# getanteon/alaz

Hardware: AMD Instinct MI355X
Metric: L7 edge-events/s ingested->scored service-map (higher is better)
Workload: dtype u64; 1 GPU; C3 device-resident replay: 10000 pods / 5000 services / 1000000 edges, 10000000 HTTP l7 events per window already in HBM, 2-layer SAGE + MLP score, partitioned K1 (variant 0, 8-byte records, 512 partitions); 2-batch HBM ring (value excludes PCIe: see end_to_end with --full); events_per_window=10000000, layers=2, windows_in_flight=1, parallelism=1 GPU

## Files before the change

alaz_amd/csrc/servicegraph.hip:

```cpp
#include <hip/hip_runtime.h>
#include <hip/hip_ext.h>

#include <algorithm>
#include <cmath>
#include <cstdio>
#include <cstring>
#include <chrono>
#include <condition_variable>
#include <thread>
#include <mutex>
#include <string>
#include <unordered_map>
#include <vector>

#include <dlfcn.h>

#include "join_host.hpp"
#include "sg_plan.hpp"
#include "sg_kernels.h"
#include "sg_sel.h"
#include "sg_trend.h"
#include "sg_node_trend.h"
#include "sg_rank.h"
#include "sg_incident.h"
// ... 160 lines not shown
    struct Impact { bool on = false; u32 max_hops = 0; sgplan::GroupImpactPlan plan; char* mem = nullptr; u32* pos = nullptr; u64* fresh = nullptr;
                    u64* next = nullptr; u64* ends = nullptr; u32* arrive = nullptr; u32* cnt = nullptr; u32* stage = nullptr; u32* stage_idx = nullptr;
                    std::vector<u64*> mask, rows, count; std::vector<u32*> hops; std::vector<char> valid; hipEvent_t ev = nullptr;
                    bool pending = false; } gimp;
    struct QuantSpace { bool on = false; char* mem = nullptr; u32* pos = nullptr; u32* tgt[2] = {nullptr, nullptr}; u64* part = nullptr;
                        unsigned char* stage = nullptr; u32* stage_idx = nullptr; std::vector<u64*> hist; std::vector<u32*> quant;
                        std::vector<char> valid; hipEvent_t ev = nullptr; bool pending = false; };
    struct Quantiles { sgplan::QuantPlan plan; u32 n_q = 0; u32 qm[SG_Q_MAX] = {}; QuantSpace sp[3]; } qnt;
    struct QuantTrend { u32 qi = 0; Baseline<sg_node_trend> nodes; Baseline<sg_edge_trend> groups; Baseline<sg_node_trend> workloads; } qtr;
    struct Traffic { double lat_floor = 0, err_floor = 0; Baseline<sg_edge_trend> edges; Baseline<sg_node_trend> nodes; Baseline<sg_edge_trend> groups;
                     Baseline<sg_node_trend> workloads; } trf;
};

namespace {

sg_engine::WinSlot& work(sg_engine* e) { return e->slots[e->cur]; }
int ran_slot(const sg_engine* e) { return e->last.slot >= 0 ? e->last.slot : e->cur; }
sg_engine::WinSlot& ran(sg_engine* e) { return e->slots[ran_slot(e)]; }

#define HIP_TRY(e, call)                                                                       \
    do {                                                                                       \
        hipError_t _r = (call);                                                                \
        if (_r != hipSuccess) {                                                                \
            (e)->err = std::string(#call) + ": " + hipGetErrorString(_r);                      \
            return _r == hipErrorOutOfMemory ? SG_ENOMEM : SG_ENODEV;                          \
        }                                                                                      \
    } while (0)

template <typename T>
int dev_alloc(sg_engine* e, T** p, size_t n, int fill = 0) {
    void* q = nullptr;
    size_t bytes = std::max<size_t>(n, 1) * sizeof(T);
    constexpr size_t kArenaMax = (size_t)32 << 20, kArenaChunk = (size_t)256 << 20, kArenaAlign = 4096;
    if (e->plan.arena_on && bytes < kArenaMax) {
        const size_t need = (bytes + kArenaAlign - 1) & ~(kArenaAlign - 1);
        if (need > e->arena_left) {
            void* c = nullptr;
            HIP_TRY(e, hipMalloc(&c, kArenaChunk));
            e->allocs.push_back(c);
            e->arena_base = static_cast<char*>(c); e->arena_left = kArenaChunk;
        }
        q = e->arena_base; e->arena_base += need; e->arena_left -= need;
    } else {
        HIP_TRY(e, hipMalloc(&q, bytes));
        e->allocs.push_back(q);
    }
    HIP_TRY(e, hipMemsetAsync(q, fill, bytes, e->slots[0].stream));
    *p = (T*)q;
    return SG_OK;
}

hipStream_t pick(sg_engine* e, void* s) { return s ? (hipStream_t)s : work(e).stream; }
hipStream_t pick_ran(sg_engine* e, void* s) { return s ? (hipStream_t)s : e->last.slot >= 0 ? e->last.stream : work(e).stream; }

hipEvent_t get_event(sg_engine* e) {
    if (!e->ev_pool.empty()) { hipEvent_t v = e->ev_pool.back(); e->ev_pool.pop_back(); return v; }
    hipEvent_t v; hipEventCreate(&v); return v;
}

struct Timed {
    sg_engine* e; hipStream_t s; TimingRec r; bool on;
    Timed(sg_engine* e_, hipStream_t s_, int kernel) : e(e_), s(s_), on(e_ && ((e_->timing >> kernel) & 1u)) {
        if (on) { r.kernel = kernel; r.a = get_event(e); r.b = get_event(e); hipEventRecord(r.a, s); }
    }
    ~Timed() { if (on) { hipEventRecord(r.b, s); e->trecs.push_back(r); } }
};

static_assert(sgplan::kK1bWarmU == K1B_WARM_U, "sg_plan.hpp's copy of pass B's warm U");
constexpr int k4_threads(int fi, bool proj, bool split) { return split ? (proj ? 512 : 256) : (fi == 32 ? 1024 : 512); }
template <class FnT, const auto& Keys> struct Family { typedef FnT Fn; static constexpr auto& keys = Keys; };
struct K1aWide : Family<K1aFn, sgplan::kK1aWideKeys> { template <size_t I> static Fn at() { constexpr auto k = keys[I]; return k1a_partition<(bool)k[0], (bool)k[1], (bool)k[2]>; } };
struct K1aTile : Family<K1aFn, sgplan::kK1aTileKeys> { template <size_t I> static Fn at() { constexpr auto k = keys[I]; return k1a_tile_partition<k[0], (bool)k[1], k[2]>; } };
struct K1aTeam : Family<K1aFn, sgplan::kK1aTeamKeys> { template <size_t I> static Fn at() { constexpr auto k = keys[I]; return k1a_team_partition<k[0], (bool)k[1], 2, 1024, k[2]>; } };
struct K1aTeamPair : Family<K1aFn, sgplan::kK1aTeamPairKeys> { template <size_t I> static Fn at() { constexpr auto k = keys[I]; return k1a_team_partition<k[0], (bool)k[1], 2, 1024, k[2], 1>; } };
struct K1bMerge : Family<K1bFn, sgplan::kK1bMergeKeys> { template <size_t I> static Fn at() {
    constexpr auto k = keys[I]; if constexpr (k[2]) return k1b_merge<k[0], (bool)k[1]>; else return k1b_merge_wide<k[0], (bool)k[1]>; } };
struct K1bStream : Family<K1bFn, sgplan::kK1bStreamKeys> { template <size_t I> static Fn at() {
    constexpr auto k = keys[I]; if constexpr (k[4]) return k1b_stream_merge<k[0], k[1], (bool)k[2], k[3]>; else return k1b_stream_merge_wide<k[0], k[1], (bool)k[2], k[3]>; } };
struct K4Layer : Family<K4LayerFn, sgplan::kK4LayerKeys> { template <size_t I> static Fn at() {
    constexpr auto k = keys[I]; return k4_sage_layer<k[0], (bool)k[1], (bool)k[2], k4_threads(k[0], k[2], k[3]), (bool)k[3]>; } };
constexpr K2RowptrFn kK2Rowptr[2] = {k2_rowptr<K2_RP_ROWS, false>, k2_rowptr<K2_RP_ROWS_DH, true>};
constexpr K4GatherFn kK4Gather[2] = {k4_gather<32>, k4_gather<64>};
constexpr K5ProjFn kK5Proj[2] = {k5_node_proj<false>, k5_node_proj<true>};
constexpr K5ScoreFn kK5Score[2][2] = {{k5_edge_score<false>, k5_edge_score<true>}, {k5_edge_score_lanes<false>, k5_edge_score_lanes<true>}};
static_assert(sgplan::kK5LanesWgLds == 4 * K5L_WAVE_LDS, "sg_plan.hpp's copy of form 1's LDS per workgroup");
template <class F, size_t... I>
const std::array<typename F::Fn, sizeof...(I)>& kernel_table(std::index_sequence<I...>) {
    static const std::array<typename F::Fn, sizeof...(I)> t{{F::template at<I>()...}};
    return t;
}
template <class F> const auto& kernel_table() { return kernel_table<F>(std::make_index_sequence<F::keys.size()>{}); }
template <class F, class... A>
typename F::Fn kernel_of(bool& ok, A... args) {
    const int i = sgplan::find_key(F::keys, sgplan::Key<sizeof...(A)>{{(int)args...}});
    if (i < 0) ok = false;
    return i < 0 ? nullptr : kernel_table<F>()[i];
}
template <class... K>
hipError_t lds_limit(size_t bytes, K... kernels) {
    for (const void* f : {reinterpret_cast<const void*>(kernels)...}) {
        const hipError_t r = hipFuncSetAttribute(f, hipFuncAttributeMaxDynamicSharedMemorySize, (int)bytes);
        if (r != hipSuccess) return r;
    }
    return hipSuccess;
}
template <class F>
hipError_t lds_limit_all(size_t bytes) { hipError_t r = hipSuccess; for (const auto f : kernel_table<F>()) if (r == hipSuccess) r = lds_limit(bytes, f); return r; }

int plan_pass_a(sg_engine* e) {
    sgplan::PassA pa = e->pa;
    if (!sgplan::plan_pass_a(e->plan, e->jt.l1_entries, e->jt.blocks_bytes(), e->ov, &pa)) { e->err = "K1 pass A: the join tables' level 1 and the piece counters do not fit a CU's LDS (fewer partitions / IP blocks needed)"; return SG_ENOSPC; }
    const sgplan::PassAKernel k = sgplan::choose_pass_a(e->plan, pa, e->cfg);
    bool ok = true;
    const K1aFn f = k.family == sgplan::K1A_TEAM ? (k.pair ? kernel_of<K1aTeamPair>(ok, k.l2, k.sharded, k.pb) : kernel_of<K1aTeam>(ok, k.l2, k.sharded, k.pb))
                  : k.family == sgplan::K1A_TILE ? kernel_of<K1aTile>(ok, k.l2, k.sharded, k.nsub) : kernel_of<K1aWide>(ok, k.l2, k.sharded, k.hist);
    if (!ok) { e->err = "K1 pass A: the library holds no kernel for family " + std::to_string(k.family) + ", level 2 mode " + std::to_string(k.l2); return SG_ENODEV; }
    e->pa = pa; e->kn.k1a = k; e->fn.k1a = f;
    return SG_OK;
}
int resolve_kernels(sg_engine* e) {
    const sgplan::Kernels& k = e->kn;
    sg_engine::Fns& f = e->fn;
    bool ok = true;
    if (k.k1b_family == sgplan::K1B_STREAM) {
        f.k1b = kernel_of<K1bStream>(ok, k.k1b_u, k.k1b_spt, k.k1b_pack, 0, k.k1b_share);
        if (k.k1b_warm) f.k1b_try = kernel_of<K1bStream>(ok, sgplan::kK1bWarmU, k.k1b_spt, k.k1b_pack, 1, k.k1b_share);
        if (k.k1b_warm) f.k1b_cold = kernel_of<K1bStream>(ok, sgplan::kK1bWarmU, k.k1b_spt, k.k1b_pack, 2, k.k1b_share);
    } else if (k.k1b_family == sgplan::K1B_MERGE) f.k1b = kernel_of<K1bMerge>(ok, k.k1b_u, k.k1b_hist, k.k1b_share);
    f.k2_rowptr = kK2Rowptr[k.k2_dh]; f.k5_proj = kK5Proj[k.k5_mfma];
    for (int w = 0; w < 2; w++) for (int pj = 0; pj < 2; pj++) f.k4_layer[w][pj] = kernel_of<K4Layer>(ok, w ? 64 : 32, k.k4_mfma, pj, k.k4_split);
    if (!ok) { e->err = "the library holds no kernel for one of the plan's choices (sg_plan.hpp choose_kernels)"; return SG_ENODEV; }
    return SG_OK;
}


void join_view(const sg_engine* e, Dev& d) {
    d.jl1mask = e->jt.l1_entries - 1;
    d.jl2_words = e->jt.use_blocks ? e->jt.blocks_used * 256u : 0u;
    d.ck_n = e->jt.ck_n;
    d.jstage_bytes = (u32)((size_t)e->jt.l1_entries * 8 + (e->pa.l2_in_lds ? e->jt.blocks_bytes() : 0));
    d.jl2_in_lds = e->pa.l2_in_lds ? 1u : 0u;
    d.k1a_ct = e->pa.k1a_ct;
}

int sync_tables(sg_engine* e, hipStream_t s) {
    sgjoin::Table& jt = e->jt;
    if (!jt.need_full && jt.dirty.empty()) return SG_OK;
    for (hipStream_t ks : e->k1_streams) if (ks != s) { HIP_TRY(e, hipEventRecord(e->k1_ev, ks)); HIP_TRY(e, hipStreamWaitEvent(s, e->k1_ev, 0)); }
    e->k1_streams.clear();
    if (jt.rebuilds == 0 && !jt.rebuild()) { e->err = "join table build failed: raise max_ips"; return SG_ENOSPC; }
    if (jt.need_full) {
        HIP_TRY(e, hipEventSynchronize(e->blob_ev));
        std::memcpy(e->h_blob, jt.blob, (size_t)jt.L.words * 4);
        HIP_TRY(e, hipMemcpyAsync(e->d_blob, e->h_blob, (size_t)jt.L.words * 4, hipMemcpyHostToDevice, s));
        HIP_TRY(e, hipEventRecord(e->blob_ev, s));
        jt.uploaded_full();
        e->st.join_full_uploads++;
    } else {
        std::vector<std::pair<u32, u32>> log;
        jt.take_dirty(log);
        std::unordered_map<u32, u32> last;
        last.reserve(log.size() * 2);
        for (auto& kv : log) last[kv.first] = kv.second;
        const int slot = e->upd_next; e->upd_next = (slot + 1) % kUpdSlots;
        HIP_TRY(e, hipEventSynchronize(e->upd_ev[slot]));
        u32 n = 0;
        for (auto& kv : last) e->h_upd[slot][n++] = make_uint2(kv.first, kv.second);
// ... 130 lines not shown
    if (dloc.warm && e->plain_left) { e->plain_left--; dloc.warm = 0; }
    w.plain = w.d.warm && !dloc.warm;
    const u32 par = w.d.k1b_par & 1u;
    if (e->plan.prepare_fold && dloc.k1b_order) { dloc.k1b_cnt += (size_t)par * dloc.np; dloc.k1b_order += (size_t)par * dloc.np; }
    const Dev& d = dloc;
    bool warm_try = d.warm && e->warm_on;
    const u32 wt = warm_try ? 1u : 0u;
    const bool fold = sgplan::close_folds(e->plan, d.warm != 0, warm_try, ob_mode);
    if (!fold) {
        Timed tp(e, s, 2);
        if (ob_mode == 1) hipLaunchKernelGGL(kc_prepare, dim3(1), dim3(1024), 0, s, d, (u64)e->n_known, (u64)e->n_labels_decl, w.ob_list, (const u32*)w.ob_n, e->plan.ob_list_cap, 1u, (const u32*)nullptr, 0u, 0u, wt);
        else if (ob_mode == 0) hipLaunchKernelGGL(kc_prepare, dim3(1), dim3(1024), 0, s, d, (u64)e->n_known, (u64)e->n_labels_decl, const_cast<u32*>(d_union), d_union_n, e->plan.ob_list_cap, 0u, (const u32*)nullptr, 0u, 0u, wt);
        else hipLaunchKernelGGL(kc_prepare, dim3(1), dim3(1024), 0, s, d, (u64)e->n_known, (u64)e->n_labels_decl, w.ob_list, (const u32*)w.ob_n, e->plan.ob_list_cap, 2u, d_union, stride, gworld, wt);
    }
    if (d.variant == 0) {
        const bool tk = ((e->timing >> 7) & 1u) && e->closes % e->timing_stride == 0;
        hipEvent_t ta = tk ? get_event(e) : nullptr, tb = tk ? get_event(e) : nullptr;
        Dev db = d; db.batch_state = w.events_in == 0 ? 2u : 0u;
        db.kept_compact = d.warm;
        const dim3 grid(d.narrow ? d.npb : d.np), block(e->plan.k1b_threads);
        if (d.warm && warm_try) {
            Dev dt = db; dim3 gt = grid;
            if (fold) {
                dt.fold = 1u; dt.warm_try = wt; gt.x += 1;
                dt.pf_n_known = (u64)e->n_known; dt.pf_n_labels_decl = (u64)e->n_labels_decl; dt.pf_list = w.ob_list; dt.pf_list_cap = e->plan.ob_list_cap;
                dt.k1b_cnt_prev = w.d.k1b_order ? w.d.k1b_cnt + (size_t)(par ^ 1u) * d.np : nullptr;
                dt.k1b_order_next = w.d.k1b_order ? w.d.k1b_order + (size_t)(par ^ 1u) * d.np : nullptr;
            }
            hipExtLaunchKernelGGL(e->fn.k1b_try, gt, block, (uint32_t)e->plan.k1b_lds, s, ta, tb, 0u, dt);
            if (tk) { TimingRec r; r.a = ta; r.b = tb; r.kernel = 7; e->trecs.push_back(r); ta = get_event(e); tb = get_event(e); }
        }
        hipExtLaunchKernelGGL(d.warm ? e->fn.k1b_cold : e->fn.k1b, grid, block, (uint32_t)e->plan.k1b_lds, s, ta, tb, 0u, db);
        if (tk) { TimingRec r; r.a = ta; r.b = tb; r.kernel = 7; e->trecs.push_back(r); }
    }
    {
        Timed t(e, s, 2);
        Dev dk = d;
        dk.kept_compact = d.warm;
        if (d.warm) {
            dk.rowptr = d.k_rowptr; dk.col = d.k_col; dk.csr_from = d.k_from; dk.acc_csr = d.k_acc; dk.max_edges = (u64)d.npb * d.pcap;
            dk.st_sum = w.scr_sum; dk.st_max = w.scr_max; dk.row_mu = w.scr_mu; dk.row_sd = w.scr_mu + d.ncap + 1;
        }
        if (d.variant == 1) {
            const u32 ntiles = e->plan.ecap / K2_TILE;
            hipLaunchKernelGGL(k2_edge_count, dim3(ntiles), dim3(256), 0, s, d);
            hipLaunchKernelGGL(k2_scan_tiles, dim3(1), dim3(1024), 0, s, d, ntiles);
            hipLaunchKernelGGL(k2_edge_compact, dim3(ntiles), dim3(256), 0, s, d);
        }
        if (d.dh_g) hipLaunchKernelGGL(k2_deg_hist, dim3(d.dh_g), dim3(K2_DH_THREADS), ((size_t)d.ncap + 1) * sizeof(u32), s, dk);
        const size_t rpr = d.dh_g ? K2_RP_ROWS_DH : K2_RP_ROWS;
        hipLaunchKernelGGL(e->fn.k2_rowptr, dim3(((size_t)d.ncap + rpr) / rpr), dim3(1024), 0, s, dk, ++e->rp_epoch);
        if (d.variant == 1) hipLaunchKernelGGL(k2_scatter_table, dim3(grid_for(e->cfg.max_edges, 256)), dim3(256), 0, s, d);
        else hipLaunchKernelGGL(k2_scatter_parts, dim3(d.npb), dim3(256), 0, s, dk);
        hipLaunchKernelGGL(k2_rowsort_gather, dim3(std::max(2, std::min(4096, 2 * K2_LONG_WGS + grid_for(d.ncap, 8)))), dim3(256), 2 * (size_t)d.k2_sortw * sizeof(u32), s, dk);
        if (d.warm) {
            const unsigned kg = (unsigned)(((u64)d.npb * d.pcap + KW_CH - 1) / KW_CH) + KW_CAPW;
            hipLaunchKernelGGL(kw_compact, dim3(kg), dim3(KW_THREADS), (size_t)KW_ROWS * 5 * sizeof(u64), s, d, ++e->kw_epoch, dk.st_sum, dk.st_max, (u64)(e->closes + 1), e->slots.size() > 1 ? 1u : 0u);
        }
    }
    {
        Timed t3(e, s, 8);
        const u32 fin = d.warm ? (u32)std::min<u64>(64, ((u64)d.ncap + 255) / 256) : 1u;
        if (fuse_in && e->plan.k3_fuse_allowed) {
            const u32 finp = d.warm ? (fin + 3) / 4 : 1u;
            hipLaunchKernelGGL(k3_in_part, dim3(e->plan.k3_ranges * e->plan.k3_slices + finp), dim3(1024), e->plan.k3in_lds, s, d, e->plan.k3_slices, finp);
            e->in_fused_slices = e->plan.k3_slices;
        } else {
            hipLaunchKernelGGL(k3_in_part, dim3(e->plan.k3_ranges * e->plan.k3_slices), dim3(1024), e->plan.k3in_lds, s, d, e->plan.k3_slices, 0u);
            hipLaunchKernelGGL(k3_in_reduce, dim3(grid_for((u64)d.ncap * 6, 256, 1024) + fin), dim3(256), 0, s, d, e->plan.k3_slices, fin);
            e->in_fused_slices = 0;
        }
    }
    HIP_TRY(e, hipGetLastError());
    w.closed = true;
    w.events_in = 0;
    e->closes++;
    if (e->plan.prepare_fold) w.d.k1b_par ^= 1u;
    return SG_OK;
}

int do_features(sg_engine* e, hipStream_t s) {
    const Dev& d = work(e).d;
    Timed t(e, s, 3);
    const int nbn = grid_for(d.ncap, 128), nbe = grid_for(e->cfg.max_edges, 256, 4096);
    hipLaunchKernelGGL(k3_node_features, dim3(nbn + nbe), dim3(256), 0, s, d, (u32)nbn, e->in_fused_slices);
    e->in_fused_slices = 0;
    HIP_TRY(e, hipGetLastError());
    return SG_OK;
}

int note_w_read(sg_engine* e, hipStream_t s) {
    for (auto& r : e->w_readers) if (r.first == s) { HIP_TRY(e, hipEventRecord(r.second, s)); return SG_OK; }
    for (size_t i = 0; i < e->w_readers.size();) {
        if (hipEventQuery(e->w_readers[i].second) == hipSuccess) { hipEventDestroy(e->w_readers[i].second); e->w_readers[i] = e->w_readers.back(); e->w_readers.pop_back(); }
        else i++;
    }
    hipEvent_t v = nullptr;
    HIP_TRY(e, hipEventCreateWithFlags(&v, hipEventDisableTiming));
    e->w_readers.emplace_back(s, v);
    HIP_TRY(e, hipEventRecord(v, s));
    return SG_OK;
}

int do_layer(sg_engine* e, u32 l, hipStream_t s, bool fuse_proj) {
    const Dev& d = work(e).d;
    if (!e->have_w) { e->err = "sg_load_weights not called"; return SG_ESTATE; }
    const float* Wl = e->d_W + layer_offset(l);
    const float* Wh = e->d_W + layer_offset(e->cfg.layers);
    const int grid = grid_for(d.ncap, 16);
    const bool pj = fuse_proj && l + 1 == e->cfg.layers && d.world == 1;
    Timed t(e, s, 4);
    const bool split = e->plan.k4_split;
    const int wide = l != 0;
    const float* hin = wide ? d.h[l] : d.x0;
    if (split) hipLaunchKernelGGL(kK4Gather[wide], dim3(grid_for(d.ncap, K4G_ROWS, 4096 * 8 / K4G_ROWS)), dim3(K4G_ROWS * 64), 0, s, d, hin);
    hipLaunchKernelGGL(e->fn.k4_layer[wide][pj], dim3(grid), dim3(k4_threads(wide ? 64 : 32, pj, split)), 0, s, d, hin, d.h[l + 1], Wl, Wh);
    HIP_TRY(e, hipGetLastError());
    return fuse_proj ? SG_OK : note_w_read(e, s);
}

template <class X>
int stage_wait(sg_engine* e, X& x, hipStream_t s) {
    if (x.pending) HIP_TRY(e, hipStreamWaitEvent(s, x.ev, 0));
    return SG_OK;
}
template <class X>
int stage_done(sg_engine* e, X& x, hipStream_t s) {
    HIP_TRY(e, hipGetLastError());
    HIP_TRY(e, hipEventRecord(x.ev, s));
    x.pending = true;
    return SG_OK;
}
NodesArgs nodes_view(const sg_engine* e, const sg_engine::WinSlot& w, u32 ncap) {
    NodesArgs a{};
    a.rows = w.d.rows; a.ctr = w.d.ctr; a.max_edges = e->cfg.max_edges;
    a.mk = w.d.max_known; a.ml = w.d.max_labels; a.mob = w.d.max_obip; a.ncap = ncap;
    return a;
}
template <class X>
void free_stage(X& x) {
    if (x.mem) { hipDeviceSynchronize(); hipFree(x.mem); }
    if (x.ev) hipEventDestroy(x.ev);
    x = X{};
}
struct StageWords { const char* off; const char* was; };
constexpr StageWords kNodesWords{"the node rollup is off (sg_set_nodes)", "the node rollup was off"};
constexpr StageWords kTrendWords{"the trend is off (sg_set_trend)", "the trend was off"};
constexpr StageWords kVanishedWords{"the vanished list is off (sg_set_vanished)", "the vanished list was off"};
constexpr StageWords kNodeTrendWords{"the node trend is off (sg_set_node_trend)", "the node trend was off"};
constexpr StageWords kRankWords{"the ranking is off (sg_set_rank)", "the ranking was off"};
constexpr StageWords kIncidentsWords{"the incidents are off (sg_set_incidents)", "the incidents were off"};
constexpr StageWords kTracksWords{"tracking is off (sg_set_tracks)", "tracking was off"};
constexpr StageWords kGroupsWords{"the groups are off (sg_set_groups)", "the groups were off"};
constexpr StageWords kGroupTrendWords{"the group trend is off (sg_set_group_trend)", "the group trend was off"};
constexpr StageWords kGroupNodesWords{"the workload rows are off (sg_set_group_nodes)", "the workload rows were off"};
constexpr StageWords kGroupNodeTrendWords{"the workload trend is off (sg_set_group_node_trend)", "the workload trend was off"};
constexpr StageWords kGroupRankWords{"the workload ranking is off (sg_set_group_rank)", "the workload ranking was off"};
constexpr StageWords kGroupIncidentsWords{"the workload incidents are off (sg_set_group_incidents)", "the workload incidents were off"};
constexpr StageWords kGroupTracksWords{"workload tracking is off (sg_set_group_tracks)", "workload tracking was off"};
constexpr StageWords kGroupImpactWords{"the workload impact is off (sg_set_group_impact)", "the workload impact was off"};
constexpr StageWords kGroupVanishedWords{"the group vanished list is off (sg_set_group_vanished)", "the group vanished list was off"};
void free_incidents(sg_engine* e);
void free_group_incidents(sg_engine* e);
struct NodeSpace {
    sg_engine::RollupState* roll; sg_engine::Baseline<sg_node_trend>* trend; sg_engine::NSel* sel; u32 cap;
    StageWords roll_w, trend_w; const char* sel_w; const char* rows_of;
    sg_engine::RankState* rank; sg_engine::IncidentState* inc; void (*inc_off)(sg_engine*);
// ... 507 lines not shown
    NodeTrendArgs a{};
    a.t = baseline_args(work(e), t);
    a.nodes = ns.roll->rows[e->cur]; a.count = ns.roll->count[e->cur]; a.ncap = ns.cap; a.out = t.rows[e->cur];
    return launch_traffic(e, t, s, a, a.t, count, write);
}
int launch_group_traffic(sg_engine* e, hipStream_t s) {
    sg_engine::Baseline<sg_edge_trend>& t = *traffic_group_edge_space(e).trend;
    GroupTrendArgs a{};
    a.t = baseline_args(work(e), t);
    a.groups = e->grp.rows[e->cur]; a.count = e->grp.count[e->cur]; a.max_edges = std::max<u64>(e->cfg.max_edges, 1); a.out = t.rows[e->cur];
    return launch_traffic(e, t, s, a, a.t, k23_gcount, k23_gwrite);
}
void free_traffic(sg_engine* e, int k) {
    if (k == kTEdges || k == kTGroups) free_baseline(k == kTEdges ? e->trf.edges : e->trf.groups);
    else free_baseline(k == kTNodes ? e->trf.nodes : e->trf.workloads);
}
void free_quantile_trend(sg_engine* e, int k) {
    if (k == kQGroups) free_baseline(e->qtr.groups);
    else free_baseline(k == kQNodes ? e->qtr.nodes : e->qtr.workloads);
}
void free_quantiles(sg_engine* e, int k) {
    free_quantile_trend(e, k);
    free_stage(e->qnt.sp[k]);
    e->qnt.plan.sp[k] = sgplan::QuantSpace{};
    e->qnt.plan.spaces &= ~(1u << k);
}
template <class Row>
void free_idxsel(sg_engine::IdxSel<Row>& s) {
    if (s.mem || s.h_n) hipDeviceSynchronize();
    if (s.mem) hipFree(s.mem);
    if (s.h_n) hipHostFree(s.h_n);
    if (s.ev) hipEventDestroy(s.ev);
    s = sg_engine::IdxSel<Row>{};
}
void free_group_nodes(sg_engine* e) {
    free_traffic(e, kTWorkloads);
    free_quantiles(e, kQWorkloads);
    free_group_incidents(e);
    free_group_rank(e);
    free_idxsel(e->gnsel);
    free_baseline(e->gntrend);
    free_stage(e->gnodes);
}

void free_groups(sg_engine* e) {
    free_group_nodes(e);
    free_traffic(e, kTGroups);
    free_quantiles(e, kQGroups);
    free_edge_trend(group_edge_space(e));
    sg_engine::Groups& x = e->grp;
    if (x.mem) hipDeviceSynchronize();
    if (x.h_up) hipHostFree(x.h_up);
    if (x.up_ev) hipEventDestroy(x.up_ev);
    free_stage(x);
}

void free_incidents(sg_engine* e) {
    free_tracks(e);
    free_stage(e->inc);
}

void free_nodes(sg_engine* e) {
    free_traffic(e, kTNodes);
    free_quantiles(e, kQNodes);
    free_incidents(e);
    free_rank(e);
    free_baseline(e->ntrend);
    free_stage(e->nodes);
}

void drop_incidents(sg_engine* e, const EdgeSpace& es) {
    const NodeSpace ns = es.nodes(e);
    if (ns.inc->on && ns.inc->p.by != SG_SEL_SCORE) ns.inc_off(e);
}

int do_score(sg_engine* e, hipStream_t s, bool proj_done, bool fuse_reset, bool* did_reset) {
    const Dev& d = work(e).d;
    if (!e->have_w) { e->err = "sg_load_weights not called"; return SG_ESTATE; }
    const float* Wh = e->d_W + layer_offset(e->cfg.layers);
    const bool fr = fuse_reset && d.variant == 0;
    {
        Timed t(e, s, 5);
        if (!(proj_done && d.world == 1)) hipLaunchKernelGGL(e->fn.k5_proj, dim3(grid_for(d.ncap, 16)), dim3(256), 0, s, d, d.h[e->cfg.layers], Wh);
        hipLaunchKernelGGL(kK5Score[e->kn.k5_form][fr], dim3((int)e->plan.k5_grid), dim3(256), 0, s, d, Wh);
    }
    if (did_reset) *did_reset = fr;
    HIP_TRY(e, hipGetLastError());
    if (const int rc = note_w_read(e, s)) return rc;
    if (e->trend.on) { const int rc = launch_trend(e, s); if (rc) return rc; }
    if (e->trf.edges.on) { if (const int rc = launch_edge_traffic(e, s)) return rc; }
    if (e->nodes.on) {
        if (const int rc = launch_nodes(e, s)) return rc;
        if (e->ntrend.on) { if (const int rc = launch_node_trend(e, node_space(e), s, k10_count, k10_write)) return rc; }
        if (e->trf.nodes.on) { if (const int rc = launch_node_traffic(e, traffic_node_space(e), s, k23_ncount, k23_nwrite)) return rc; }
        if (e->rank.on) { if (const int rc = launch_rank(e, s)) return rc; }
        if (e->inc.on) { if (const int rc = launch_incidents(e, s)) return rc; }
        if (e->trk.on) { if (const int rc = launch_node_tracks(e, s)) return rc; }
        if (e->qnt.sp[kQNodes].on) { if (const int rc = launch_quantiles(e, kQNodes, s)) return rc; }
        if (e->qtr.nodes.on) { if (const int rc = launch_node_tail(e, tail_node_space(e), kQNodes, s, k21_ncount, k21_nwrite)) return rc; }
    }
    if (e->grp.on) {
        if (const int rc = launch_groups(e, s)) return rc;
        if (e->gtrend.on) { if (const int rc = launch_group_trend(e, s)) return rc; }
        if (e->trf.groups.on) { if (const int rc = launch_group_traffic(e, s)) return rc; }
        if (e->qnt.sp[kQGroups].on) { if (const int rc = launch_quantiles(e, kQGroups, s)) return rc; }
        if (e->qtr.groups.on) { if (const int rc = launch_group_tail(e, s)) return rc; }
        if (e->gnodes.on) {
            if (const int rc = launch_group_nodes(e, s)) return rc;
            if (e->gntrend.on) { if (const int rc = launch_node_trend(e, workload_space(e), s, k16_tcount, k16_twrite)) return rc; }
            if (e->trf.workloads.on) { if (const int rc = launch_node_traffic(e, traffic_workload_space(e), s, k23_wcount, k23_wwrite)) return rc; }
            if (e->grank.on) { if (const int rc = launch_group_rank(e, s)) return rc; }
            if (e->ginc.on) { if (const int rc = launch_group_incidents(e, s)) return rc; }
            if (e->gtrk.on) { if (const int rc = launch_group_tracks(e, s)) return rc; }
            if (e->gimp.on) { if (const int rc = launch_group_impact(e, s)) return rc; }
            if (e->qnt.sp[kQWorkloads].on) { if (const int rc = launch_quantiles(e, kQWorkloads, s)) return rc; }
            if (e->qtr.workloads.on) { if (const int rc = launch_node_tail(e, tail_workload_space(e), kQWorkloads, s, k21_wcount, k21_wwrite)) return rc; }
        }
    }
    return SG_OK;
}

int do_reset(sg_engine* e, hipStream_t s) {
    sg_engine::WinSlot& w = work(e);
    hipLaunchKernelGGL(k_reset_window, dim3(grid_for(std::max<u64>((u64)w.d.ncap * SG_NODE_STAT_SUM_WORDS, e->plan.obcap), 256, 512)), dim3(256), 0, s, w.d);
    HIP_TRY(e, hipGetLastError());
    w.closed = false;
    w.events_in = 0;
    return SG_OK;
}

void window_timed_end(sg_engine* e, hipStream_t s) {
    if (!e->win_ta) return;
    TimingRec r; r.kernel = 10; r.a = e->win_ta; r.b = get_event(e);
    hipEventRecord(r.b, s);
    e->trecs.push_back(r);
    e->win_ta = nullptr;
}

void account_window(sg_engine* e) {
    sg_engine::WinSlot& w = work(e);
    const size_t E = (size_t)e->h_ctr[C_N_EDGES];
    sg_stats& st = e->st;
    st.windows++;
    st.last_window_events = e->h_ctr[C_N_EVENTS];
    st.last_window_edges = E;
    st.last_window_nodes = e->h_ctr[C_N_NODES];
    st.events_dropped_src += e->h_ctr[C_DROPPED_SRC];
    st.events_dropped_cap += e->h_ctr[C_DROPPED_CAP];
    st.events_misrouted += e->h_ctr[C_MISROUTED];
    {
        const u64 h = e->h_ctr[C_HALO_OVF];
        st.halo_overflow += h - w.halo_ovf_seen;
        w.halo_ovf_seen = h;
    }
    st.alive_in += e->h_ctr[C_ALIVE_SEEN];
    st.alive_dropped += e->h_ctr[C_ALIVE_DROPPED];
    st.last_window_new_edges = 0;
    if (w.d.warm && w.plain) st.windows_plain++;
    else if (w.d.warm) {
        const bool cold = e->h_ctr[C_LAST_COLD] != 0;
        if (cold) st.windows_cold++; else st.windows_warm++;
        if (!cold && e->h_ctr[C_LAST_DELTA]) { st.windows_delta++; st.last_window_new_edges = e->h_ctr[C_LAST_DELTA]; }
    }
    if (e->h_ctr[C_N_EVENTS]) {
        st.last_window_tmin_ms = (int64_t)((e->first_user - (e->first_kernel - e->h_ctr[C_TMIN_NS])) / 1000000ull);
        st.last_window_tmax_ms = (int64_t)((e->first_user - (e->first_kernel - e->h_ctr[C_TMAX_NS])) / 1000000ull);
    } else { st.last_window_tmin_ms = st.last_window_tmax_ms = 0; }
// ... 722 lines not shown
    }
    e->kn = sgplan::choose_kernels(P, e->pa, *cfg);
    CR(resolve_kernels(e));
    CH(lds_limit(2 * (size_t)d.k2_sortw * sizeof(u32), k2_rowsort_gather));
    if (d.dh_g) CH(lds_limit(((size_t)d.ncap + 1) * sizeof(u32), k2_deg_hist));
    CH(lds_limit(P.k3in_lds, k3_in_part));
    CR(dev_alloc(e, &d.dbg, (size_t)4 * 4096 * 8));
    CR(dev_alloc(e, &d.clk, (size_t)4));
    CR(dev_alloc(e, &e->d_W, weights_count(cfg->layers)));
    d.W = e->d_W;
    {
        float* tab = nullptr;
        CR(dev_alloc(e, &tab, (size_t)SG_L1P_TAB));
        hipLaunchKernelGGL(k_l1p_table, dim3((SG_L1P_TAB + 255) / 256), dim3(256), 0, e->slots[0].stream, tab);
        CH(hipStreamSynchronize(e->slots[0].stream));
        d.l1p_tab = tab;
    }
    auto alloc_window = [&](sg_engine::WinSlot& slot) -> int {
        Dev& w = slot.d;
#define LR(call) do { int _rc = (call); if (_rc) return _rc; } while (0)
        size_t eslots = ME;
        if (w.variant == 0) {
            eslots = std::max<size_t>(ME, (size_t)w.npb * w.pcap);
            if (w.narrow) { LR(dev_alloc(e, &w.slab8, (size_t)w.np * w.nwg * w.punits)); LR(dev_alloc(e, &w.hdr8, (size_t)w.np * w.nwg));
                            if (P.k1b_order) {
                                const size_t halves = P.prepare_fold ? 2 : 1;
                                LR(dev_alloc(e, &w.k1b_cnt, halves * w.np)); LR(dev_alloc(e, &w.k1b_order, halves * w.np));
                                std::vector<u32> ident(halves * w.np);
                                for (size_t i = 0; i < ident.size(); i++) ident[i] = (u32)(i % w.np);
                                HIP_TRY(e, hipStreamSynchronize(e->slots[0].stream));
                                HIP_TRY(e, hipMemcpy(w.k1b_order, ident.data(), ident.size() * sizeof(u32), hipMemcpyHostToDevice));
                            } }
            else { LR(dev_alloc(e, &w.slab_s, (size_t)w.np * w.nwg * w.pslots)); LR(dev_alloc(e, &w.hdr, (size_t)w.np * w.nwg)); }
            LR(dev_alloc(e, &w.ovf, (size_t)w.ovf_cap * 9));
            LR(dev_alloc(e, &w.ovf_p, (size_t)w.ovf_cap));
            LR(dev_alloc(e, &w.part_n, w.npb));
            LR(dev_alloc(e, &w.acc_src, (size_t)w.npb * w.pcap * 4));
            LR(dev_alloc(e, &w.e_rank, (size_t)w.npb * w.pcap));
            if (w.dh_g) LR(dev_alloc(e, &w.dh_hist, (size_t)w.dh_g * w.dh_ns));
            if (w.warm) {
                const size_t KC = (size_t)w.npb * w.pcap;
                LR(dev_alloc(e, &w.wk_keys, (size_t)w.npb * w.k1b_ht, 0xFF)); LR(dev_alloc(e, &w.wk_pos, (size_t)w.npb * w.k1b_ht, 0xFF));
                LR(dev_alloc(e, &w.pos_of_slot, KC, 0xFF));
                LR(dev_alloc(e, &w.k_acc, KC * 4)); LR(dev_alloc(e, &w.k_col, KC)); LR(dev_alloc(e, &w.k_from, KC)); LR(dev_alloc(e, &w.k_rowptr, (size_t)w.ncap + 2));
                LR(dev_alloc(e, &w.kw_tot, (KC + KW_CH - 1) / KW_CH + 2));
                LR(dev_alloc(e, &w.k_col2, KC)); LR(dev_alloc(e, &w.k_from2, KC)); LR(dev_alloc(e, &w.k_rowptr2, (size_t)w.ncap + 2));
                LR(dev_alloc(e, &w.k_slot, 2 * KC));
                LR(dev_alloc(e, &w.dc_rowptr, (size_t)w.ncap + 2)); LR(dev_alloc(e, &w.dc_col, KC)); LR(dev_alloc(e, &w.dc_from, KC)); LR(dev_alloc(e, &w.dc_acc, KC * 4));
                LR(dev_alloc(e, &w.dc_slot, KC)); LR(dev_alloc(e, &w.dc_ip, KC)); LR(dev_alloc(e, &w.dl_img, KC));
                LR(dev_alloc(e, &w.deg2, ((size_t)w.ncap + 1) * SG_DEG_REP * SG_DEG_STRIDE));
                LR(dev_alloc(e, &slot.scr_sum, (size_t)w.ncap * SG_NODE_STAT_SUM_WORDS)); LR(dev_alloc(e, &slot.scr_max, (size_t)w.ncap * SG_NODE_STAT_MAX_WORDS)); LR(dev_alloc(e, &slot.scr_mu, 2 * ((size_t)w.ncap + 1)));
                void* dn = nullptr;
                HIP_TRY(e, hipHostMalloc((void**)&slot.h_note, 64, hipHostMallocMapped));
                slot.h_note[0] = slot.h_note[1] = 0;
                HIP_TRY(e, hipHostGetDevicePointer(&dn, slot.h_note, 0));
                w.host_note = (u64*)dn;
            }
        }
        const size_t KE = P.kept_edges;
        LR(dev_alloc(e, &w.ekeys, P.ecap, 0xFF));
        LR(dev_alloc(e, &w.eacc, (size_t)P.ecap * 4));
        if (w.variant == 1) w.acc_src = w.eacc;
        LR(dev_alloc(e, &w.obkeys, P.obcap));
        LR(dev_alloc(e, &w.wgstat, (size_t)SG_MAX_K1_WGS * WS_WORDS));
        LR(dev_alloc(e, &w.ctr, C_COUNT));
        LR(dev_alloc(e, &w.ob_sorted, w.max_obip));
        LR(dev_alloc(e, &slot.ob_list, P.ob_list_cap));
        LR(dev_alloc(e, &slot.ob_n, 4));
        LR(dev_alloc(e, &w.tile_cnt, P.ecap / K2_TILE));
        LR(dev_alloc(e, &w.tile_off, P.ecap / K2_TILE));
        LR(dev_alloc(e, &w.e_slot, ME)); LR(dev_alloc(e, &w.e_from, eslots)); LR(dev_alloc(e, &w.e_to, eslots));
        LR(dev_alloc(e, &w.longrows, (size_t)w.ncap + 1));
        LR(dev_alloc(e, &w.deg, ((size_t)w.ncap + 1) * SG_DEG_REP * SG_DEG_STRIDE)); LR(dev_alloc(e, &w.rp_tot, ((size_t)w.ncap + K2_RP_ROWS_DH) / K2_RP_ROWS_DH + 1)); LR(dev_alloc(e, &w.k6_tot, (((size_t)w.ncap + 1023) / 1024 + 1) * 16)); LR(dev_alloc(e, &w.k1a_ticket, 4)); LR(dev_alloc(e, &w.lb_ticket, 4)); w.k1a_ticket_base = 0; w.k1a_rot = 0; LR(dev_alloc(e, &w.rowptr, (size_t)w.ncap + 1)); LR(dev_alloc(e, &w.cursor, (size_t)w.ncap + 1));
        LR(dev_alloc(e, &w.col, ME)); LR(dev_alloc(e, &w.cs, KE)); LR(dev_alloc(e, &w.csr_from, ME));
        LR(dev_alloc(e, &w.sort_k, 2 * KE)); LR(dev_alloc(e, &w.sort_v, 2 * KE));
        LR(dev_alloc(e, &w.acc_csr, ME * 4));
        if (w.hist) { LR(dev_alloc(e, &w.hist_src, (w.variant == 0 ? (size_t)w.npb * w.pcap : (size_t)P.ecap) * SG_HIST_BINS)); LR(dev_alloc(e, &w.hist_csr, ME * SG_HIST_BINS)); }
        LR(dev_alloc(e, &w.st_sum, (size_t)w.ncap * SG_NODE_STAT_SUM_WORDS)); LR(dev_alloc(e, &w.st_max, (size_t)w.ncap * SG_NODE_STAT_MAX_WORDS));
        LR(dev_alloc(e, &w.x0, (size_t)w.ncap * SG_F_IN));
        for (u32 l = 1; l <= cfg->layers; l++) LR(dev_alloc(e, &w.h[l], (size_t)w.ncap * SG_F_HID));
        LR(dev_alloc(e, &w.P, (size_t)w.ncap * SG_F_HID)); LR(dev_alloc(e, &w.Q, (size_t)w.ncap * SG_F_HID));
        LR(dev_alloc(e, &w.nmean, (size_t)w.ncap * SG_F_HID));
        LR(dev_alloc(e, &w.hub_items, w.hub_cap)); LR(dev_alloc(e, &w.hub_base, (size_t)w.ncap + 1)); LR(dev_alloc(e, &w.hub_part, (size_t)w.hub_cap * SG_F_HID));
        LR(dev_alloc(e, &w.efeat, ME * SG_F_EDGE)); LR(dev_alloc(e, &w.latz, ME)); LR(dev_alloc(e, &w.errr, ME));
        LR(dev_alloc(e, &w.row_mu, (size_t)w.ncap + 1)); LR(dev_alloc(e, &w.row_sd, (size_t)w.ncap + 1));
        LR(dev_alloc(e, &w.rows, ME));
        LR(dev_alloc(e, &w.in_part, (size_t)P.k3_ranges * P.k3_slices * K3_IN_NR * 6));
        LR(dev_alloc(e, &w.alive_keys, w.alive_cap)); LR(dev_alloc(e, &w.alive_csr, KE));
        LR(dev_alloc(e, &w.act_l, (size_t)w.ncap + 1)); LR(dev_alloc(e, &w.act_p, (size_t)w.ncap + 1));
        std::vector<u64> init((size_t)SG_MAX_K1_WGS * WS_WORDS, 0);
        for (int i = 0; i < SG_MAX_K1_WGS; i++) init[(size_t)i * WS_WORDS + WS_TMIN] = ~0ull;
        HIP_TRY(e, hipMemcpy(w.wgstat, init.data(), init.size() * sizeof(u64), hipMemcpyHostToDevice));
#undef LR
        return SG_OK;
    };
    CH(hipStreamSynchronize(e->slots[0].stream));
    for (sg_engine::WinSlot& slot : e->slots) {
        slot.d = base;
        if (!slot.stream) CH(hipStreamCreateWithFlags(&slot.stream, hipStreamNonBlocking));
        CR(alloc_window(slot));
    }
    CH(hipStreamCreateWithFlags(&e->copy_stream, hipStreamNonBlocking)); CH(hipStreamCreateWithFlags(&e->copy_stream2, hipStreamNonBlocking));
    CH(hipStreamCreateWithFlags(&e->rd_stream, hipStreamNonBlocking)); CH(hipEventCreateWithFlags(&e->score_ev, hipEventDisableTiming));
    CH(hipHostMalloc((void**)&e->h_ctr_pin, sizeof(e->h_ctr)));
    for (int i = 0; i < P.n_stage; i++) {
        CH(hipEventCreateWithFlags(&e->copied_ev[i], hipEventDisableTiming));
        CH(hipHostMalloc((void**)&e->h_stage[i], (size_t)e->cfg.max_batch * sizeof(sg_event)));
        CR(dev_alloc(e, &e->d_stage[i], e->cfg.max_batch));
        CH(hipEventCreateWithFlags(&e->stage_ev[i], hipEventDisableTiming));
    }
    CH(hipDeviceSynchronize());
#undef CR
#undef CH
    *out = e;
    return SG_OK;
}

int sg_destroy(sg_handle e) {
    if (!e) return SG_EINVAL;
    hipDeviceSynchronize();
    for (sg_engine::WinSlot& w : e->slots) { if (w.stream) hipStreamDestroy(w.stream); if (w.h_note) hipHostFree(w.h_note); }
    for (void* p : e->allocs) hipFree(p);
    if (e->h_blob) hipHostFree(e->h_blob);
    for (int i = 0; i < kUpdSlots; i++) { if (e->h_upd[i]) hipHostFree(e->h_upd[i]); if (e->upd_ev[i]) hipEventDestroy(e->upd_ev[i]); }
    if (e->blob_ev) hipEventDestroy(e->blob_ev);
    if (e->k1_ev) hipEventDestroy(e->k1_ev);
    for (int i = 0; i < kStageSlots; i++) { if (e->h_stage[i]) hipHostFree(e->h_stage[i]); if (e->stage_ev[i]) hipEventDestroy(e->stage_ev[i]); if (e->copied_ev[i]) hipEventDestroy(e->copied_ev[i]); }
    for (auto& r : e->registered) hipHostUnregister(const_cast<char*>(r.first));
    if (e->copy_stream) hipStreamDestroy(e->copy_stream);
    if (e->copy_stream2) hipStreamDestroy(e->copy_stream2);
    if (e->rd_stream) hipStreamDestroy(e->rd_stream);
    if (e->score_ev) hipEventDestroy(e->score_ev);
    for (auto& r : e->w_readers) hipEventDestroy(r.second);
    if (e->h_ctr_pin) hipHostFree(e->h_ctr_pin);
    if (e->h_rows) hipHostFree(e->h_rows);
    if (e->h_rows_old) hipHostFree(e->h_rows_old);
    if (e->sel.stage) hipFree(e->sel.stage);
    if (e->sel.stage_idx) hipFree(e->sel.stage_idx);
    if (e->sel.h_n) hipHostFree(e->sel.h_n);
    if (e->sel.ev) hipEventDestroy(e->sel.ev);
    free_edge_trend(edge_space(e));
    free_traffic(e, kTEdges);
    free_nodes(e);
    free_groups(e);
    free_idxsel(e->nsel);
    free_idxsel(e->gsel);
    for (auto& r : e->trecs) { hipEventDestroy(r.a); hipEventDestroy(r.b); }
    for (auto v : e->ev_pool) hipEventDestroy(v);
    if (e->tab_ev) hipEventDestroy(e->tab_ev);
    delete e;
    return SG_OK;
}

int sg_geometry_get(sg_handle e, sg_geometry* out) {
    if (!e || !out) return SG_EINVAL;
    std::lock_guard<std::mutex> g(e->mu);
    const sgplan::Plan& p = e->plan; const sgplan::PassA& a = e->pa;
    out->k1_variant = p.variant; out->k1_narrow = p.narrow; out->partitions = p.np; out->table_slots = p.k1b_ht; out->pass_b_split = p.k1b_split;
    out->pass_a_workgroups = p.nwg; out->cache_slots = a.k1a_ct; out->join_l2_in_lds = a.l2_in_lds ? (p.narrow && a.l2_u16 ? 2u : 1u) : 0u;
    out->tile_records = p.narrow ? (a.k1a_team ? 4u * a.k1a_nt / a.k1a_teams : K1T_TS(a.k1a_nsub)) : 0u; out->pass_a_teams = p.narrow && a.k1a_team ? a.k1a_teams : 0u; out->endpoint_bits = p.narrow ? p.nb : 0u;
    out->piece_bytes = p.variant != 0 ? 0u : (p.narrow ? p.punits * 8u : p.pslots * 16u);
    out->warm_windows = p.warm;
    return SG_OK;
}

int sg_prepare_fold_get(sg_handle e, uint32_t* out) {
    if (!e || !out) return SG_EINVAL;
    std::lock_guard<std::mutex> g(e->mu);
    *out = e->plan.prepare_fold ? 1u : 0u;
    return SG_OK;
}

int sg_pass_a_pair_get(sg_handle e, uint32_t* out) {
    if (!e || !out) return SG_EINVAL;
    std::lock_guard<std::mutex> g(e->mu);
    *out = e->plan.narrow && e->pa.k1a_team && e->pa.k1a_pair ? 1u : 0u;
    return SG_OK;
}

int sg_k5_form_get(sg_handle e, uint32_t* out) {
    if (!e || !out) return SG_EINVAL;
    std::lock_guard<std::mutex> g(e->mu);
    *out = (uint32_t)e->kn.k5_form;
    return SG_OK;
}

int sg_upsert_pod(sg_handle e, uint32_t ip, uint32_t node_id) {
    if (!e) return SG_EINVAL;
    std::lock_guard<std::mutex> g(e->mu);
    return table_upsert(e, false, ip, node_id, SG_NODE_POD);
}
int sg_upsert_service(sg_handle e, uint32_t ip, uint32_t node_id) {
    if (!e) return SG_EINVAL;
    std::lock_guard<std::mutex> g(e->mu);
    return table_upsert(e, true, ip, node_id, SG_NODE_SERVICE);
}
int sg_delete_pod(sg_handle e, uint32_t ip) {
    if (!e) return SG_EINVAL;
    std::lock_guard<std::mutex> g(e->mu);
    if (!e->jt.erase(false, ip)) { e->err = "join table rebuild failed"; return SG_ENOSPC; }
    return SG_OK;
}
int sg_delete_service(sg_handle e, uint32_t ip) {
    if (!e) return SG_EINVAL;
    std::lock_guard<std::mutex> g(e->mu);
    if (!e->jt.erase(true, ip)) { e->err = "join table rebuild failed"; return SG_ENOSPC; }
    return SG_OK;
}

int sg_set_clock(sg_handle e, uint64_t first_kernel_ns, uint64_t first_user_ns) {
    if (!e) return SG_EINVAL;
    std::lock_guard<std::mutex> g(e->mu);
    e->first_kernel = first_kernel_ns; e->first_user = first_user_ns;
    return SG_OK;
}

int sg_set_label_count(sg_handle e, uint32_t n_labels) {
    if (!e) return SG_EINVAL;
    std::lock_guard<std::mutex> g(e->mu);
    if (n_labels > e->cfg.max_labels) { e->err = "label count beyond max_labels"; return SG_ENOSPC; }
    e->n_labels_decl = std::max(e->n_labels_decl, n_labels);
    return SG_OK;
}

int sg_load_weights(sg_handle e, const float* w, size_t n) {
    if (!e || !w) return SG_EINVAL;
    std::lock_guard<std::mutex> g(e->mu);
    if (n != weights_count(e->cfg.layers)) { e->err = "weight count mismatch"; return SG_EINVAL; }
    for (auto& r : e->w_readers) HIP_TRY(e, hipEventSynchronize(r.second));
    for (auto& r : e->w_readers) hipEventDestroy(r.second);
    e->w_readers.clear();
    HIP_TRY(e, hipMemcpy(e->d_W, w, n * sizeof(float), hipMemcpyHostToDevice));
    e->have_w = true;
    return SG_OK;
}

namespace {
int stage_take(sg_engine* e) {
    for (int k = 0; k < e->plan.n_stage; k++) {
        const int c = (e->stage_next + k) % e->plan.n_stage;
        if (!e->stage_busy[c] && hipEventQuery(e->stage_ev[c]) != hipErrorNotReady) { e->stage_busy[c] = true; e->stage_next = (c + 1) % e->plan.n_stage; e->pending_copies++; return c; }
    }
    return -1;
}
hipStream_t stage_stream(sg_engine* e) { return (e->plan.n_copy == 2 && (e->copy_rr++ & 1)) ? e->copy_stream2 : e->copy_stream; }
int stage_finish(sg_engine* e, int slot, size_t n, hipStream_t cs, bool copy_ok) {
    sg_engine::WinSlot& w = work(e);
    int rc = SG_OK;
    if (!copy_ok) { e->err = "hipMemcpyAsync (staging ring)"; rc = SG_ENODEV; }
    if (rc == SG_OK) {
        hipEventRecord(e->copied_ev[slot], cs);
        hipStreamWaitEvent(w.stream, e->copied_ev[slot], 0);
        e->st.h2d_bytes += n * sizeof(sg_event);
        rc = launch_k1(e, e->d_stage[slot], n, w.stream);
    }
    hipEventRecord(e->stage_ev[slot], w.stream);
    e->stage_busy[slot] = false; e->pending_copies--;
    e->cv.notify_all();
    return rc;
}
int stage_submit(sg_engine* e, int slot, const sg_event* src, size_t n) {
    hipStream_t cs = stage_stream(e);
    const bool ok = hipMemcpyAsync(e->d_stage[slot], src, n * sizeof(sg_event), hipMemcpyHostToDevice, cs) == hipSuccess;
    return stage_finish(e, slot, n, cs, ok);
}
constexpr size_t kStagePiece = ((size_t)4 << 20) / sizeof(sg_event);
// ... 1791 lines not shown
```

alaz_amd/csrc/sg_k2.h:

```cpp
#pragma once

__device__ __forceinline__ void kc_warm_decide(const Dev& d, u32 warm_try, u64 n_known, u64 nl, u64 nob) {
    if (!d.warm) return;
    (void)n_known; (void)nl;
    const bool ok = warm_try && d.ctr[C_KEPT_VALID] && d.ctr[C_KEPT_E] != 0 && nob == 0;
    d.ctr[C_COLD] = ok ? 0ull : 1ull;
}
struct KcScratch {
    u64 red[7][16];
    u64 nkl;
    u64 nl_s;
    __attribute__((aligned(16))) u32 hb[256];
    u32 wsum[17];
    u32 cnt, cmax;
};
template <bool FOLD>
__device__ __forceinline__ void kc_prepare_rest(const Dev& d, KcScratch& sc, u64 n_known, u64 n_labels_decl, u32* list, const u32* n_in, u32 list_cap, u32 collect,
                                                const u32* seg, u32 seg_stride, u32 seg_world, u32 warm_try, u32* cnt_io, u32* order_out) {
    u64 (&red)[7][16] = sc.red; u32 (&wsum)[17] = sc.wsum; u32& cnt = sc.cnt; u64& nkl = sc.nkl; u64& nl_s = sc.nl_s;
    const u32 t = threadIdx.x, lane = t & 63, wave = t >> 6;
    const u64 ob0 = (!FOLD && collect == 1 && t <= d.obmask) ? d.obkeys[t] : 0ull;
    const u64 nl_prev = (!FOLD && t == 0) ? d.ctr[C_N_LABELS] : 0ull;
    {
        u64 tmin = ~0ull, tmax = 0, ml = 0, ds = 0, dc = 0, mr = 0, ac = 0;
// ... 389 lines not shown
            const u64 pos = (u64)rp[q] + dg[q] + rk[q];
            if (i0 + 256u * q < n && pos < d.max_edges) d.cs[pos] = make_uint2(to[q], slot[q]);
        }
    }
}

__device__ __forceinline__ double mean_us(u64 sum_ns, u64 cnt) { return cnt ? ((double)sum_ns / 1000.0) / (double)cnt : 0.0; }
__device__ __forceinline__ double std_us(u64 sum_ns, u64 ssq_us, u64 cnt) {
    if (!cnt) return 0.0;
    const double m = mean_us(sum_ns, cnt);
    const double v = (double)ssq_us / (double)cnt - m * m;
    return v > 0.0 ? sqrt(v) : 0.0;
}

struct EdgeEmitArgs { u64* acc_csr; u32* csr_from; u64* eacc; u64* ekeys; u32* alive_csr; u32 variant; u32* hist_src; u32* hist_csr; u32 hist; u32* pos_of_slot; u32* slot_of_pos; };
__device__ __forceinline__ void edge_emit(const EdgeEmitArgs d, u32 pos, u32 row, u32 slot, u64, u64, u64, const ulonglong2 x, const ulonglong2 y) {
    ulonglong2* dst = reinterpret_cast<ulonglong2*>(d.acc_csr + (size_t)pos * 4);
    dst[0] = x; dst[1] = y;
    d.csr_from[pos] = row;
    if (d.pos_of_slot) d.pos_of_slot[slot] = pos;
    if (d.slot_of_pos) d.slot_of_pos[pos] = slot;
    d.alive_csr[pos] = 0;
    if (d.hist) {
        uint4* hs = reinterpret_cast<uint4*>(d.hist_src + (size_t)slot * SG_HIST_BINS); uint4* hd = reinterpret_cast<uint4*>(d.hist_csr + (size_t)pos * SG_HIST_BINS);
        const uint4 h0 = hs[0], h1 = hs[1], h2 = hs[2], h3 = hs[3];
        hd[0] = h0; hd[1] = h1; hd[2] = h2; hd[3] = h3;
        if (d.variant == 1) { const uint4 z = make_uint4(0, 0, 0, 0); hs[0] = z; hs[1] = z; hs[2] = z; hs[3] = z; }
    }
    if (d.variant == 1) {
        ulonglong2* src = reinterpret_cast<ulonglong2*>(d.eacc + (size_t)slot * 4);
        src[0] = make_ulonglong2(0, 0); src[1] = make_ulonglong2(0, 0);
        d.ekeys[slot] = SG_EKEY_EMPTY;
    }
}
__global__ __launch_bounds__(256) void k_clock_spin(u64* clk, u32 iters) {
    u32 a = threadIdx.x, b = a * 3u + 1u, c = a * 5u + 7u;
    const u64 c0 = __builtin_readcyclecounter(), r0 = wall_clock64();
    for (u32 i = 0; i < iters; i++) { a = a * 1664525u + b; b = b * 22695477u + c; c ^= a >> 3; }
    const u64 c1 = __builtin_readcyclecounter(), r1 = wall_clock64();
    if (threadIdx.x == 0 && blockIdx.x == 0) { clk[2] = c1 - c0; clk[3] = r1 - r0; }
    if ((a ^ b ^ c) == 0x12345678u) clk[3] = a;
}
#define SG_CHASE_A 0x9E3779B5u
#define SG_CHASE_C 0x7F4A7C15u
__global__ __launch_bounds__(256) void k_chase_init(u32* buf, u32 mask) {
    for (u64 x = (u64)blockIdx.x * 256 + threadIdx.x; x <= mask; x += (u64)gridDim.x * 256) buf[x * 32] = ((u32)x * SG_CHASE_A + SG_CHASE_C) & mask;
    if (blockIdx.x == 0 && threadIdx.x == 0) buf[1] = mask;
}
__device__ __forceinline__ u32 out_mask(const u32* buf) { return buf[1]; }
__global__ void k_chase(const u32* buf, u32 steps, u64* out) {
    const u32 mask_start = (blockIdx.x * blockDim.x + threadIdx.x) * 0x9E3779B1u;
    u32 x = (gridDim.x * blockDim.x) == 1 ? 0u : (mask_start & out_mask(buf));
    const u64 t0 = wall_clock64();
    for (u32 i = 0; i < steps; i++) x = __builtin_nontemporal_load(buf + (size_t)x * 32);
    const u64 t1 = wall_clock64();
    if (blockIdx.x == 0 && threadIdx.x == 0) out[0] = t1 - t0;
    if (x == 0xFFFFFFFFu) out[1] = x;
}
__global__ void k_l1p_table(float* tab) { const u32 i = blockIdx.x * blockDim.x + threadIdx.x; if (i < SG_L1P_TAB) tab[i] = (float)log1p((double)i); }
__device__ __forceinline__ float log1p_count(const Dev& d, u64 c) { return c < SG_L1P_TAB ? d.l1p_tab[c] : (float)log1p((double)c); }
__device__ __forceinline__ double sg_rcp(double d) {
    double r = __builtin_amdgcn_rcp(d);
    double e = fma(-d, r, 1.0); r = fma(r, e, r);
    e = fma(-d, r, 1.0); return fma(r, e, r);
}
__device__ __forceinline__ double sg_div(double n, double d) { const double r = sg_rcp(d), q = n * r; return fma(fma(-d, q, n), r, q); }
__device__ __forceinline__ double sg_log1p_pos(double x) {
    const double y = 1.0 + x;
    double m = __builtin_amdgcn_frexp_mant(y);
    int e = __builtin_amdgcn_frexp_exp(y);
    const bool lo = m < 0.70710678118654752;
    m = lo ? m + m : m; e = lo ? e - 1 : e;
    const double s = sg_div(m - 1.0, m + 1.0), s2 = s * s;
    double p = 1.0 / 19.0;
    p = fma(p, s2, 1.0 / 17.0); p = fma(p, s2, 1.0 / 15.0); p = fma(p, s2, 1.0 / 13.0); p = fma(p, s2, 1.0 / 11.0);
    p = fma(p, s2, 1.0 / 9.0); p = fma(p, s2, 1.0 / 7.0); p = fma(p, s2, 1.0 / 5.0); p = fma(p, s2, 1.0 / 3.0);
    const double logm = fma(2.0 * s * s2, p, 2.0 * s);
    const double c = (x - (y - 1.0)) * sg_rcp(y);
    const double ed = (double)e;
    const double r = fma(ed, 6.93147180369123816490e-01, logm + fma(ed, 1.90821492927058770002e-10, c));
    const double sm = x * (1.0 - x * (0.5 - x * (1.0 / 3.0 - 0.25 * x)));
    return x < 1e-4 ? sm : r;
}
__device__ __forceinline__ void edge_features(const Dev& d, u32 pos) {
    const ulonglong2* a = reinterpret_cast<const ulonglong2*>(d.acc_csr + (size_t)pos * 4);
    const ulonglong2 x = a[0], y = a[1];
    const u32 from = d.csr_from[pos];
    const u64 cnt = x.x & 0xFFFFFFFFull, err = x.x >> 32, sum = x.y, mx = y.x, ssq = y.y;
    const double rc = cnt ? sg_rcp((double)cnt) : 0.0, dc = (double)cnt;
    const double sum_us = (double)sum * 1e-3;
    double m_e = sum_us * rc; m_e = cnt ? fma(fma(-dc, m_e, sum_us), rc, m_e) : 0.0;
    double q_e = (double)ssq * rc; q_e = cnt ? fma(fma(-dc, q_e, (double)ssq), rc, q_e) : 0.0;
    const double var = q_e - m_e * m_e, s_e = var > 0.0 ? sqrt(var) : 0.0;
    const double mu = d.row_mu[from], sd = d.row_sd[from];
    const double z = sd > 1.0 ? sg_div(m_e - mu, sd) : m_e - mu;
    const float lat_z = (float)z;
    const float err_ratio = !cnt ? 0.0f : ((cnt | err) < (1ull << 24) ? (float)(u32)err / (float)(u32)cnt : (float)((double)err / (double)cnt));
    const float zc = lat_z < -8.0f ? -8.0f : (lat_z > 8.0f ? 8.0f : lat_z);
    float4* e = reinterpret_cast<float4*>(d.efeat + (size_t)pos * SG_F_EDGE);
    e[0] = make_float4(log1p_count(d, cnt), (float)sg_log1p_pos(m_e * 1e-3), (float)sg_log1p_pos(s_e * 1e-3), (float)sg_log1p_pos((double)mx * 1e-6));
    e[1] = make_float4(err_ratio, log1p_count(d, err), zc * 0.125f, 1.0f);
    d.latz[pos] = lat_z; d.errr[pos] = err_ratio;
}

#define K2_LONG_WGS 1024
#define K2_WAVE_ROW 512
#define K2_WAVE_BW  1024
__device__ __forceinline__ void k2_row_wg(const Dev& d, const EdgeEmitArgs& ea, const u32 rr, u32* sk, u32* sv, u64 (*red)[4], u32* bsum, const u32 BW) {
    const u32 lane = threadIdx.x & 63, wave = threadIdx.x >> 6;
    const u32 b = d.rowptr[rr];
    u32 m = d.rowptr[rr + 1] - b;
    if ((u64)b + m > d.max_edges) m = b < d.max_edges ? (u32)(d.max_edges - b) : 0;
    if (m == 0) return;
    const uint2* in = d.cs + b; u32* key = d.col + b;
    u64 cnt = 0, err = 0, sum = 0, ssq = 0, mx = 0;
    if (BW <= d.k2_sortw && m <= 1024) {
        for (u32 w = threadIdx.x; w < BW; w += 256) sk[w] = 0;
        __syncthreads();
        u32 mk[4], mv[4]; ulonglong2 ax[4], ay[4];
#pragma unroll
        for (int q = 0; q < 4; q++) {
            const u32 i = threadIdx.x + q * 256;
            const uint2 kv = in[i < m ? i : m - 1]; mk[q] = i < m ? kv.x : 0u; mv[q] = i < m ? kv.y : 0u;
        }
#pragma unroll
        for (int q = 0; q < 4; q++) {
            const u32 i = threadIdx.x + q * 256;
            if (i < m) { atomicOr(&sk[mk[q] >> 5], 1u << (mk[q] & 31)); const ulonglong2* a = reinterpret_cast<const ulonglong2*>(d.acc_src + (size_t)mv[q] * 4); ax[q] = a[0]; ay[q] = a[1]; }
            else { ax[q] = make_ulonglong2(0, 0); ay[q] = make_ulonglong2(0, 0); }
        }
        __syncthreads();
        {
            const u32 per = (BW + 255) / 256, w0 = threadIdx.x * per < BW ? threadIdx.x * per : BW, w1 = w0 + per < BW ? w0 + per : BW;
            u32 c = 0;
            for (u32 w = w0; w < w1; w++) c += __popc(sk[w]);
            u32 tot;
            u32 run = block_excl_scan<256>(c, bsum, &tot);
            for (u32 w = w0; w < w1; w++) { sv[w] = run; run += __popc(sk[w]); }
        }
        __syncthreads();
#pragma unroll
        for (int q = 0; q < 4; q++) { cnt += ax[q].x & 0xFFFFFFFFull; err += ax[q].x >> 32; sum += ax[q].y; ssq += ay[q].y; mx = ay[q].x > mx ? ay[q].x : mx; }
#pragma unroll
        for (int q = 0; q < 4; q++) if (threadIdx.x + q * 256 < m) {
            const u32 k = mk[q], r = sv[k >> 5] + __popc(sk[k >> 5] & ((1u << (k & 31)) - 1u));
            key[r] = k;
            edge_emit(ea, b + r, rr, mv[q], 0, 0, 0, ax[q], ay[q]);
        }
        cnt = wave_sum_u64(cnt); err = wave_sum_u64(err); sum = wave_sum_u64(sum); ssq = wave_sum_u64(ssq); mx = wave_max_u64(mx);
        if (lane == 0) { red[0][wave] = cnt; red[1][wave] = err; red[2][wave] = sum; red[3][wave] = ssq; red[4][wave] = mx; }
        __syncthreads();
        cnt = red[0][0] + red[0][1] + red[0][2] + red[0][3]; err = red[1][0] + red[1][1] + red[1][2] + red[1][3];
        sum = red[2][0] + red[2][1] + red[2][2] + red[2][3]; ssq = red[3][0] + red[3][1] + red[3][2] + red[3][3];
        mx = red[4][0]; for (int w = 1; w < 4; w++) mx = red[4][w] > mx ? red[4][w] : mx;
    } else if (BW <= d.k2_sortw) {
        for (u32 w = threadIdx.x; w < BW; w += 256) sk[w] = 0;
        __syncthreads();
        for (u32 i0 = 0; i0 < m; i0 += 1024) {
            u32 k4[4];
#pragma unroll
            for (int q = 0; q < 4; q++) { const u32 i = i0 + threadIdx.x + q * 256; k4[q] = in[i < m ? i : m - 1].x; }
#pragma unroll
            for (int q = 0; q < 4; q++) if (i0 + threadIdx.x + q * 256 < m) atomicOr(&sk[k4[q] >> 5], 1u << (k4[q] & 31));
        }
        __syncthreads();
        {
            const u32 per = (BW + 255) / 256, w0 = threadIdx.x * per < BW ? threadIdx.x * per : BW, w1 = w0 + per < BW ? w0 + per : BW;
            u32 c = 0;
            for (u32 w = w0; w < w1; w++) c += __popc(sk[w]);
            u32 tot;
            u32 run = block_excl_scan<256>(c, bsum, &tot);
            for (u32 w = w0; w < w1; w++) { sv[w] = run; run += __popc(sk[w]); }
        }
        __syncthreads();
        for (u32 i0 = 0; i0 < m; i0 += 1024) {
            u32 k4[4], v4[4]; ulonglong2 x4[4], y4[4];
#pragma unroll
            for (int q = 0; q < 4; q++) { const u32 i = i0 + threadIdx.x + q * 256; const uint2 kv = in[i < m ? i : m - 1]; k4[q] = kv.x; v4[q] = kv.y; }
#pragma unroll
            for (int q = 0; q < 4; q++) { const ulonglong2* a = reinterpret_cast<const ulonglong2*>(d.acc_src + (size_t)v4[q] * 4); x4[q] = a[0]; y4[q] = a[1]; }
#pragma unroll
            for (int q = 0; q < 4; q++) if (i0 + threadIdx.x + q * 256 < m) {
                const u32 k = k4[q], r = sv[k >> 5] + __popc(sk[k >> 5] & ((1u << (k & 31)) - 1u));
                key[r] = k;
                edge_emit(ea, b + r, rr, v4[q], 0, 0, 0, x4[q], y4[q]);
                cnt += x4[q].x & 0xFFFFFFFFull; err += x4[q].x >> 32; sum += x4[q].y; ssq += y4[q].y; mx = y4[q].x > mx ? y4[q].x : mx;
// ... 315 lines not shown
```

alaz_amd/csrc/sg_k5.h:

```cpp
#pragma once

template <bool USE_MFMA>
__global__ __launch_bounds__(256) void k5_node_proj(Dev d, const float* __restrict__ hL, const float* __restrict__ Wh) {
    constexpr int LDA = SG_F_HID + 2;
    __shared__ float A[16 * LDA];
    __shared__ u32 vid[16];
    const bool listed = d.world > 1 && d.ctr[C_ACT_L] != SG_ACT_NONE;
    const u32 N = listed ? (u32)d.ctr[C_ACT_P] : (u32)d.ctr[C_N_NODES];
    const float* __restrict__ Wu = Wh; const float* __restrict__ Wv = Wh + SG_F_HID * SG_F_HID;
    const float* __restrict__ b1 = Wv + SG_F_HID * SG_F_HID + SG_F_EDGE * SG_F_HID;
    const u32 wave = threadIdx.x >> 6, lane = threadIdx.x & 63;
    for (u32 tile = blockIdx.x; tile * 16 < N; tile += gridDim.x) {
        const u32 v0 = tile * 16;
        if (threadIdx.x < 16) vid[threadIdx.x] = v0 + threadIdx.x < N ? (listed ? d.act_p[v0 + threadIdx.x] : v0 + threadIdx.x) : 0u;
        __syncthreads();
        for (u32 idx = threadIdx.x; idx < 16 * SG_F_HID; idx += 256) {
            const u32 r = idx >> 6, k = idx & 63;
            A[r * LDA + k] = (v0 + r < N) ? hL[(size_t)vid[r] * SG_F_HID + k] : 0.0f;
        }
        __syncthreads();
        if (USE_MFMA) {
            const int jb = wave * 16, i = lane & 15;
            const float bj = b1[jb + i];
            f32x4 p = { bj, bj, bj, bj }, q = { 0.0f, 0.0f, 0.0f, 0.0f };
// ... 80 lines not shown
            x = x > 0.0f ? x : 0.0f;
            r[m] = x * w2r[m];
        }
        float sum = (r[0] + r[2]) + (r[1] + r[3]);
        sum = sum + xor_partner_f32(sum, 8); sum = sum + xor_partner_f32(sum, 4);
        sum = sum + xor_partner_f32(sum, 2); sum = sum + xor_partner_f32(sum, 1);
        return sum;
    };
    static_assert(SG_F_EDGE == 8, "k5_edge_score spreads two 8-float edge feature vectors over a DPP row of 16 lanes");
    const u32* __restrict__ idsrc = (q & 1u) ? d.col : d.csr_from;
    const u32 wk = lane & 7u, we8 = lane >> 3;
    const u32* __restrict__ srcA = wk == 3 ? d.csr_from : reinterpret_cast<const u32*>(d.errr);
    const u32* __restrict__ srcB = wk == 3 ? d.col : (wk == 5 ? reinterpret_cast<const u32*>(d.latz) : d.alive_csr);
    const u32 accj = wk < 3 ? wk + 1 : 0u;
    const int srcl = (int)(((we8 & 3u) << 4) | (we8 < 4 ? 0u : 8u));
    if (E) {
        const u32 stride = nw * 8, last = E - 1;
        u32 pa = wave * 8 + g, pb = pa + 4;
        struct K5Set { float4 PA, QA, PB, QB; u32 ew, wa, wb; u64 wacc; };
        auto ids_of = [&](u32 xa, u32 xb) -> u32 { const u32 px = (q & 2u) ? xb : xa; return idsrc[px < E ? px : last]; };
        auto issue = [&](u32 idw_, u32 xa, u32 xb, u32 x0, K5Set& S) {
            u32 ua = dpp32b<0x150>(idw_), va = dpp32b<0x151>(idw_), ub = dpp32b<0x152>(idw_), vb = dpp32b<0x153>(idw_);
            if SG_ABL(d, 0x1000u) { ua &= 15u; va &= 15u; ub &= 15u; vb &= 15u; }
            const u32 ca = xa < E ? xa : last, cb = xb < E ? xb : last;
            S.PA = reinterpret_cast<const float4*>(d.P + (size_t)ua * SG_F_HID)[q]; S.QA = reinterpret_cast<const float4*>(d.Q + (size_t)va * SG_F_HID)[q];
            S.PB = reinterpret_cast<const float4*>(d.P + (size_t)ub * SG_F_HID)[q]; S.QB = reinterpret_cast<const float4*>(d.Q + (size_t)vb * SG_F_HID)[q];
            S.ew = __float_as_uint(d.efeat[(size_t)(q < 8 ? ca : cb) * SG_F_EDGE + (q & 7u)]);
            const u32 er_ = x0 + we8, ec_ = er_ < E ? er_ : last;
            S.wacc = d.acc_csr[(size_t)ec_ * 4 + accj];
            S.wa = srcA[ec_]; S.wb = srcB[ec_];
        };
        auto iter = [&](K5Set& cur, K5Set& nxt, const u32 idw_next, u32& idw_after, const u32 p0) {
            const u32 na = pa + stride, nb = pb + stride;
            idw_after = ids_of(na + stride, nb + stride);
            issue(idw_next, na, nb, p0 + stride, nxt);
            __builtin_amdgcn_sched_barrier(0);
            const float4 PA = cur.PA, QA = cur.QA, PB = cur.PB, QB = cur.QB;
            const u32 ew = cur.ew, wa = cur.wa, wb = cur.wb; const u64 wacc = cur.wacc;
            const u32 er = p0 + we8, ec = er < E ? er : last;
            const float eka[SG_F_EDGE] = {__uint_as_float(dpp32b<0x150>(ew)), __uint_as_float(dpp32b<0x151>(ew)), __uint_as_float(dpp32b<0x152>(ew)), __uint_as_float(dpp32b<0x153>(ew)),
                                          __uint_as_float(dpp32b<0x154>(ew)), __uint_as_float(dpp32b<0x155>(ew)), __uint_as_float(dpp32b<0x156>(ew)), __uint_as_float(dpp32b<0x157>(ew))};
            const float ekb[SG_F_EDGE] = {__uint_as_float(dpp32b<0x158>(ew)), __uint_as_float(dpp32b<0x159>(ew)), __uint_as_float(dpp32b<0x15A>(ew)), __uint_as_float(dpp32b<0x15B>(ew)),
                                          __uint_as_float(dpp32b<0x15C>(ew)), __uint_as_float(dpp32b<0x15D>(ew)), __uint_as_float(dpp32b<0x15E>(ew)), __uint_as_float(dpp32b<0x15F>(ew))};
            const float sa = step(PA, QA, eka);
            const float sb = step(PB, QB, ekb);
            const float mysum = __shfl(q < 8 ? sa : sb, srcl, 64);
            u64 val = wacc;
            if (wk == 3) val = (u64)ref_of_dense(wa, nk, nl) | ((u64)ref_of_dense(wb, nk, nl) << 32);
            else if (wk == 5) { const float logit = mysum + b2; val = (u64)__float_as_uint(1.0f / (1.0f + expf(-logit))) | ((u64)wb << 32); }
            else if (wk == 6) val = (u64)wa | ((u64)wb << 32);
            else if (wk == 7) {
                val = 0;
                if (d.hist) {
                    const ulonglong2* __restrict__ ac = reinterpret_cast<const ulonglong2*>(d.acc_csr + (size_t)ec * 4);
                    val = k5_percentiles(d, ec, (u32)(ac[0].x & 0xFFFFFFFFull), ac[1].x);
                }
            }
            {
                const u32 p0u = (u32)__builtin_amdgcn_readfirstlane((int)p0);
                const u32 nrow = SG_ABL(d, 0x2000u) ? 0u : (E - p0u < 8u ? E - p0u : 8u);
                const __amdgpu_buffer_rsrc_t rr_ = __builtin_amdgcn_make_buffer_rsrc(reinterpret_cast<u64*>(d.rows) + (size_t)p0u * 8, 0, (int)(nrow * 64u), 0x00020000);
                v2u_t dv; dv.x = (u32)val; dv.y = (u32)(val >> 32);
                __builtin_amdgcn_raw_buffer_store_b64(dv, rr_, lane * 8u, 0, 0);
            }
            pa = na; pb = nb;
        };
        K5Set A, B;
        u32 i1 = ids_of(pa + stride, pb + stride), i2;
        { const u32 id0 = ids_of(pa, pb); issue(id0, pa, pb, wave * 8, A); }
        for (u32 p0 = wave * 8; p0 < E; p0 += 2 * stride) {
            iter(A, B, i1, i2, p0);
            if (p0 + stride >= E) break;
            iter(B, A, i2, i1, p0 + stride);
        }
    }
    if (RESET) k5_window_reset(d);
}

typedef float f32x2 __attribute__((ext_vector_type(2)));
typedef u32 v4u_t __attribute__((ext_vector_type(4)));
#define K5L_WAVE_LDS 8192u
__device__ __forceinline__ void k5l_lds_order() { __builtin_amdgcn_fence(__ATOMIC_ACQ_REL, "wavefront"); __builtin_amdgcn_wave_barrier(); }

template <bool RESET>
__global__ __launch_bounds__(256) __attribute__((amdgpu_waves_per_eu(3))) void k5_edge_score_lanes(Dev d, const float* __restrict__ Wh) {
#pragma clang fp contract(off)
    static_assert(SG_F_HID == 64 && SG_F_EDGE == 8, "k5_edge_score_lanes: 64 hidden units in four quarters, eight edge features");
    __shared__ __attribute__((aligned(256))) f32x4 lds[4 * K5L_WAVE_LDS / 16];
    const u32 E = (u32)d.ctr[C_N_EDGES], nk = (u32)d.ctr[C_N_KNOWN], nl = (u32)d.ctr[C_N_LABELS];
    const float* __restrict__ We = Wh + 2 * SG_F_HID * SG_F_HID;
    const float* __restrict__ w2 = We + SG_F_EDGE * SG_F_HID + SG_F_HID;
    const float b2 = w2[SG_F_HID];
    const u32 lane = threadIdx.x & 63;
    const u32 wave = (blockIdx.x * 256 + threadIdx.x) >> 6, nw = (gridDim.x * 256) >> 6;
    f32x4* const tile = lds + (threadIdx.x >> 6) * (K5L_WAVE_LDS / 16);
    if (E) {
        const u32 last = E - 1, nbatch = (E + 63u) >> 6;
        const u32 sub = lane >> 2, pc = lane & 3u;
        const u32 wslot = sub * 4 + (pc ^ ((sub >> 2) & 3u));
        const u32 rx = (lane >> 2) & 3u;
        const u32 ox = (lane >> 1) & 3u;
        const u32 rb = (((lane >> 3) * 4 + (((lane & 7u) >> 1) ^ ((lane >> 4) & 3u))) << 1) | (lane & 1u);
        u32 gu[4], gv[4];
        f32x4 R[8];
        auto load_ids = [&](u32 p0) {
#pragma unroll
            for (int i = 0; i < 4; i++) { const u32 p = p0 + i * 16 + sub, c = p < E ? p : last; gu[i] = d.csr_from[c]; gv[i] = d.col[c]; }
        };
        auto row_offsets = [&]() {
#pragma unroll
            for (int i = 0; i < 4; i++) { gu[i] = gu[i] * (SG_F_HID * 4u) + pc * 16u; gv[i] = gv[i] * (SG_F_HID * 4u) + pc * 16u; }
        };
        auto issue = [&](int c) {
#pragma unroll
            for (int i = 0; i < 4; i++) {
                R[i] = *reinterpret_cast<const f32x4*>(reinterpret_cast<const char*>(d.P) + gu[i] + c * 64);
                R[4 + i] = *reinterpret_cast<const f32x4*>(reinterpret_cast<const char*>(d.Q) + gv[i] + c * 64);
            }
        };
        float S[8];
        float ek[SG_F_EDGE];
        auto quarter = [&](int c, float (&out)[4]) {
            f32x4 pq[4];
#pragma unroll
            for (int w = 0; w < 4; w++) pq[w] = tile[(lane * 4 + rx) ^ (u32)w] + tile[256 + ((lane * 4 + rx) ^ (u32)w)];
            f32x4 W[2][4], w2v[4];
            auto wload = [&](int blk, f32x4 (&dst)[4]) {
                u32 o = (u32)((blk & 1) * 4 * SG_F_HID + 16 * (blk >> 1) + 4 * c);
                asm volatile("" : "+s"(o));
#pragma unroll
                for (int i = 0; i < 4; i++) dst[i] = *reinterpret_cast<const f32x4*>(We + o + i * SG_F_HID);
            };
            wload(0, W[0]);
            f32x2 xa[4], xb[4], ta, tb;
#pragma unroll
            for (int blk = 0; blk < 8; blk++) {
                const int m = blk >> 1, kh = blk & 1;
                __builtin_amdgcn_s_waitcnt(0xC07F);
                if (blk < 7) wload(blk + 1, W[(blk + 1) & 1]);
                else {
                    u32 o = (u32)(4 * c);
                    asm volatile("" : "+s"(o));
#pragma unroll
                    for (int i = 0; i < 4; i++) w2v[i] = *reinterpret_cast<const f32x4*>(w2 + o + 16 * i);
                }
                __builtin_amdgcn_sched_barrier(0);
                if (kh == 0) { ta = (f32x2){ pq[0][m], pq[1][m] }; tb = (f32x2){ pq[2][m], pq[3][m] }; }
#pragma unroll
                for (int i = 0; i < 4; i++) {
                    const f32x2 ee = { ek[kh * 4 + i], ek[kh * 4 + i] };
                    ta = __builtin_elementwise_fma(ee, W[blk & 1][i].xy, ta);
                    tb = __builtin_elementwise_fma(ee, W[blk & 1][i].zw, tb);
                }
                if (kh == 1) { ta = __builtin_elementwise_max(ta, (f32x2){ 0.0f, 0.0f }); tb = __builtin_elementwise_max(tb, (f32x2){ 0.0f, 0.0f }); }
                asm volatile("" : "+v"(ta), "+v"(tb));
                if (kh == 1) { xa[m] = ta; xb[m] = tb; }
                __builtin_amdgcn_sched_barrier(0);
            }
            __builtin_amdgcn_s_waitcnt(0xC07F);
            const f32x2 sa = __builtin_elementwise_fma(w2v[0].xy, xa[0], w2v[2].xy * xa[2]) + __builtin_elementwise_fma(w2v[1].xy, xa[1], w2v[3].xy * xa[3]);
            const f32x2 sb = __builtin_elementwise_fma(w2v[0].zw, xb[0], w2v[2].zw * xb[2]) + __builtin_elementwise_fma(w2v[1].zw, xb[1], w2v[3].zw * xb[3]);
            out[0] = sa.x; out[1] = sa.y; out[2] = sb.x; out[3] = sb.y;
        };
        u32 b = wave;
        if (b < nbatch) { load_ids(b * 64u); row_offsets(); issue(0); }
        for (; b < nbatch; b += nw) {
            const u32 p0 = b * 64u;
            const u32 er = p0 + lane, ec = er < E ? er : last;
            const u32 np0 = b + nw < nbatch ? (b + nw) * 64u : last;
            const f32x4 e0 = reinterpret_cast<const f32x4*>(d.efeat + (size_t)ec * SG_F_EDGE)[0], e1 = reinterpret_cast<const f32x4*>(d.efeat + (size_t)ec * SG_F_EDGE)[1];
            float T[4];
#define K5L_STAGE(C, NEXT) { k5l_lds_order();                                                                                \
                _Pragma("unroll") for (int i = 0; i < 4; i++) { tile[64 * i + wslot] = R[i]; tile[256 + 64 * i + wslot] = R[4 + i]; } \
                k5l_lds_order(); NEXT; __builtin_amdgcn_sched_barrier(0); }
            K5L_STAGE(0, issue(2))
            ek[0] = e0[0]; ek[1] = e0[1]; ek[2] = e0[2]; ek[3] = e0[3]; ek[4] = e1[0]; ek[5] = e1[1]; ek[6] = e1[2]; ek[7] = e1[3];
            { float o[4]; quarter(0, o); S[0] = o[0]; S[1] = o[1]; S[2] = o[2]; S[3] = o[3]; }
            K5L_STAGE(2, issue(1))
            { float o[4]; quarter(2, o); for (int i = 0; i < 4; i++) S[i] = S[i] + o[i]; }
            K5L_STAGE(1, { issue(3); load_ids(np0); })
            { float o[4]; quarter(1, o); S[4] = o[0]; S[5] = o[1]; S[6] = o[2]; S[7] = o[3]; }
            const ulonglong2 a01 = reinterpret_cast<const ulonglong2*>(d.acc_csr + (size_t)ec * 4)[0], a23 = reinterpret_cast<const ulonglong2*>(d.acc_csr + (size_t)ec * 4)[1];
            const u32 mu = d.csr_from[ec], mv = d.col[ec];
            const u32 wer = reinterpret_cast<const u32*>(d.errr)[ec], wlz = reinterpret_cast<const u32*>(d.latz)[ec], wal = d.alive_csr[ec];
            K5L_STAGE(3, { row_offsets(); issue(0); })
            { float o[4]; quarter(3, o); for (int i = 0; i < 4; i++) S[4 + i] = S[4 + i] + o[i]; }
#undef K5L_STAGE
#pragma unroll
            for (int i = 0; i < 4; i++) T[i] = S[i] + S[4 + i];
            const float sum = (T[0] + T[2]) + (T[1] + T[3]);
            const float logit = sum + b2;
            const u32 score = __float_as_uint(1.0f / (1.0f + expf(-logit)));
            const u64 refs = (u64)ref_of_dense(mu, nk, nl) | ((u64)ref_of_dense(mv, nk, nl) << 32);
            u64 pct = 0;
            if (d.hist) pct = k5_percentiles(d, ec, (u32)(a01.x & 0xFFFFFFFFull), a23.x);
            v4u_t* const ot = reinterpret_cast<v4u_t*>(tile);
            k5l_lds_order();
            ot[(lane * 4 + ox) ^ 0u] = (v4u_t){ (u32)a01.y, (u32)(a01.y >> 32), (u32)a23.x, (u32)(a23.x >> 32) };
            ot[(lane * 4 + ox) ^ 1u] = (v4u_t){ (u32)a23.y, (u32)(a23.y >> 32), (u32)refs, (u32)(refs >> 32) };
            ot[(lane * 4 + ox) ^ 2u] = (v4u_t){ (u32)a01.x, (u32)(a01.x >> 32), score, wlz };
            ot[(lane * 4 + ox) ^ 3u] = (v4u_t){ wer, wal, (u32)pct, (u32)(pct >> 32) };
            k5l_lds_order();
            {
                const u32 p0u = (u32)__builtin_amdgcn_readfirstlane((int)p0);
                const u32 nrow = SG_ABL(d, 0x2000u) ? 0u : (E - p0u < 64u ? E - p0u : 64u);
                const __amdgpu_buffer_rsrc_t rr_ = __builtin_amdgcn_make_buffer_rsrc(reinterpret_cast<u64*>(d.rows) + (size_t)p0u * 8, 0, (int)(nrow * 64u), 0x00020000);
                const v2u_t* const rt = reinterpret_cast<const v2u_t*>(tile);
#pragma unroll
                for (int j = 0; j < 8; j++) __builtin_amdgcn_raw_buffer_store_b64(rt[64 * j + rb], rr_, (u32)j * 512u + lane * 8u, 0, 0);
            }
        }
    }
    if (RESET) k5_window_reset(d);
}
```

alaz_amd/csrc/sg_plan.hpp:

```cpp
#pragma once
#include <algorithm>
#include <array>
#include <cmath>
#include <cstdint>
#include <cstdlib>
#include <cstring>
#include <initializer_list>
#include <optional>
#include <string>
#include <vector>

#include "../../include/servicegraph.h"
#include "sg_sizes.h"

namespace sgplan {

typedef uint32_t u32;
typedef uint64_t u64;

constexpr size_t kLdsBytes = 160 * 1024;
constexpr int kStageSlots = 32;
constexpr size_t kPrepareLds = 4096;

inline u32 next_pow2(u64 v) { u64 p = 1; while (p < v) p <<= 1; return (u32)p; }
inline int grid_for(u64 items, int per_block, int cap = 2048) {
    u64 g = (items + per_block - 1) / per_block;
    return (int)std::max<u64>(1, std::min<u64>(g, (u64)cap));
}

struct DeviceFacts {
    int cus = 256;
    size_t lds_bytes = kLdsBytes;
};

struct Overrides {
    typedef std::optional<std::string> Knob;
    Knob ablate, np, ht, ct, nwg, nsub, split, warm, k1a, k1_narrow, k1_legacy, k1b_u, k1b_threads, k1b_pack, k1b_no_order,
         l2_global, l2_u32, dh_g, k3_slices, k3_no_fuse, k4_fused, k5_grid, k6_one_wg, dense_valu, copy_streams, stage_slots, arena, no_fold, k1a_pair, k5_form;
};
struct KnobName { const char* name; Overrides::Knob Overrides::*field; };
constexpr KnobName kKnobs[] = {
    {"SG_ABLATE", &Overrides::ablate}, {"SG_NP", &Overrides::np}, {"SG_HT", &Overrides::ht}, {"SG_CT", &Overrides::ct},
    {"SG_NWG", &Overrides::nwg}, {"SG_NSUB", &Overrides::nsub}, {"SG_SPLIT", &Overrides::split}, {"SG_WARM", &Overrides::warm},
    {"SG_K1A", &Overrides::k1a}, {"SG_K1_NARROW", &Overrides::k1_narrow}, {"SG_K1_LEGACY", &Overrides::k1_legacy},
    {"SG_K1B_U", &Overrides::k1b_u}, {"SG_K1B_THREADS", &Overrides::k1b_threads}, {"SG_K1B_PACK", &Overrides::k1b_pack},
    {"SG_K1B_NO_ORDER", &Overrides::k1b_no_order}, {"SG_L2_GLOBAL", &Overrides::l2_global}, {"SG_L2_U32", &Overrides::l2_u32},
    {"SG_DH_G", &Overrides::dh_g}, {"SG_K3_SLICES", &Overrides::k3_slices}, {"SG_K3_NO_FUSE", &Overrides::k3_no_fuse},
    {"SG_K4_FUSED", &Overrides::k4_fused}, {"SG_K5_GRID", &Overrides::k5_grid}, {"SG_K6_ONE_WG", &Overrides::k6_one_wg},
    {"SG_DENSE_VALU", &Overrides::dense_valu}, {"SG_COPY_STREAMS", &Overrides::copy_streams}, {"SG_STAGE_SLOTS", &Overrides::stage_slots},
    {"SG_ARENA", &Overrides::arena}, {"SG_NO_FOLD", &Overrides::no_fold}, {"SG_K1A_PAIR", &Overrides::k1a_pair},
    {"SG_K5_FORM", &Overrides::k5_form},
};
#ifdef SG_DEV_KNOBS
inline Overrides from_env() {
    Overrides o;
    for (const KnobName& k : kKnobs) if (const char* v = std::getenv(k.name)) o.*k.field = std::string(v);
    return o;
}
#endif
inline int ival(const Overrides::Knob& k) { return std::atoi(k->c_str()); }
inline u64 uval(const Overrides::Knob& k) { return std::strtoull(k->c_str(), nullptr, 0); }

struct Plan {
    u32 variant = 0, narrow = 0, hist = 0, agg_slots = 3, nb = 0, np = 0, pb = 0, nwg = 256, k1b_split = 1, k1b_ht = 0, npb = 0, rb = 0,
        pcap = 0, sa = 0, sn = 0, sw = 0, punits = 0, ss = 0, pslots = 0, ovf_cap = 0, warm = 0;
    u32 k1b_threads = 1024, k1b_u = 4;
    bool k1b_pack = false;
    bool k1b_order = false;
    size_t k1b_lds = 0;
    bool prepare_fold = false;
    u32 ecap = 0, obcap = 0, ob_list_cap = 0, ncap = 0, max_obip = 1, alive_cap = 0, hub_cap = 0, max_blocks = 0;
    u64 kept_edges = 0;
    u32 max_known = 0;
    u32 k3_ranges = 1, k3_slices = 8;
    size_t k3in_lds = 0;
    u32 k2_sortw = 0, dh_g = 0, dh_ppw = 0, dh_ns = 0;
    bool k4_split = false;
    u32 k5_grid = 0;
    u32 k5_form = 0;
    bool k3_fuse_allowed = true;
    bool k6_one_wg = false;
    bool use_mfma = true;
    u32 cus = 1;
    int k1_grid = 0, n_copy = 1, n_stage = 16;
    bool arena_on = false;
    u32 n_slots = 1;
    u32 ablate = 0;
};

struct PassA {
    bool l2_u16 = false, k1a_team = false, l2_in_lds = false;
    u32 k1a_nsub = 2, k1a_teams = 2, k1a_nt = 1024, k1a_ct = 2048;
    size_t k1a_lds = 0;
    bool k1a_pair = false;
    size_t k1a_pair_lds = 0;
};

inline int check_config(const sg_config& in, sg_config* out) {
    constexpr uint32_t kCfgMin = 88;
    if (in.struct_size < kCfgMin || in.struct_size > 4096) return SG_EINVAL;
    sg_config c; std::memset(&c, 0, sizeof c);
    std::memcpy(&c, &in, std::min<size_t>(in.struct_size, sizeof c));
    c.struct_size = (uint32_t)sizeof c;
    if (c.abi_version != SG_ABI_VERSION || c.layers < 1 || c.layers > SG_MAX_LAYERS || c.max_edges == 0 ||
        c.max_known_nodes == 0 || c.world == 0 || c.rank >= c.world || c.max_known_nodes > 0x3FFFFFFFu)
        return SG_EINVAL;
    if (c.max_batch == 0) c.max_batch = 1u << 20;
    if (c.max_ips == 0) c.max_ips = c.max_known_nodes;
    if (c.max_window_events == 0) c.max_window_events = c.max_batch;
    *out = c;
    return SG_OK;
}

constexpr u64 kK5LanesMinEdges = 1ull << 20;
inline u32 k5_form_default(const sg_config& cfg) { return cfg.world <= 1 && cfg.max_edges >= kK5LanesMinEdges ? 1u : 0u; }
constexpr size_t kK5LanesWgLds = 4 * 8192;
constexpr int kK5LanesWaves = 3;
constexpr int k5_lanes_wgs_per_cu() { return (int)std::min<size_t>(kLdsBytes / kK5LanesWgLds, (size_t)kK5LanesWaves); }
inline int make_plan(const sg_config& cfg, const DeviceFacts& dev, const Overrides& ov, Plan* out, std::string* why) {
    sg_config chk;
    if (check_config(cfg, &chk) != SG_OK) { if (why) *why = "invalid config"; return SG_EINVAL; }
    Plan p;
    const size_t lds = dev.lds_bytes;
    if (ov.arena) p.arena_on = ival(ov.arena) != 0;
    p.k1_grid = std::min<int>(SG_MAX_K1_WGS, dev.cus * 8);
    p.cus = (u32)std::max(1, dev.cus);
    p.use_mfma = !(ov.dense_valu && (*ov.dense_valu)[0] == '1');
    p.max_known = cfg.max_known_nodes;

    const u64 ME = cfg.max_edges;
    p.ecap = next_pow2(std::max<u64>(2 * ME, K2_TILE));
    p.obcap = next_pow2(std::max<u64>(2 * (u64)cfg.max_outbound_ips, 64));
    p.ob_list_cap = next_pow2(std::max<u64>((u64)cfg.max_outbound_ips * std::max<u32>(cfg.world, 1), 64));
    p.max_obip = std::max<u32>(cfg.max_outbound_ips, 1);
    p.ncap = cfg.max_known_nodes + cfg.max_labels + p.max_obip;

    p.variant = cfg.k1_variant == 1 ? 1u : 0u;
    p.hist = (cfg.flags & SG_CFG_EDGE_HISTOGRAM) ? 1u : 0u;
    p.agg_slots = p.hist ? 5u : 3u;
    const u64 cn = (u64)cfg.max_known_nodes + cfg.max_labels + p.obcap;
    u32 nb = 12; while ((1ull << nb) < cn && nb < 31) nb++;
    bool narrow = p.variant == 0 && !p.hist && cfg.k1_variant != 2 && !ov.k1_legacy && nb <= 24;
    const bool small_window = ME < (1ull << 18) && cfg.max_window_events <= (2ull << 20);
    if (cfg.k1_variant == 0 && small_window && !ov.k1_narrow) narrow = false;
    u64 np = 0;
    if (narrow) {
        np = next_pow2(std::max<u64>((ME + 2699) / 2700, 256));
        u32 pbt = 0; while ((1ull << pbt) < np) pbt++;
        if (np > 2048 || 2 * nb - pbt > 31) narrow = false;
    }
    p.k1b_split = 1;
    if (narrow) {
        if (ME / np > 1150) { p.k1b_split = 2; p.k1b_ht = 2048; }
        else p.k1b_ht = ME / np > 550 ? 2048 : 1024;
        if (ov.split) { const int x = ival(ov.split); if (x == 1 || x == 2) { p.k1b_split = (u32)x; p.k1b_ht = ME / (np * x) > 1150 ? 4096 : (ME / (np * x) > 550 ? 2048 : 1024); } }
    } else {
        np = next_pow2(std::max<u64>((ME + 1249) / 1250, 256));
        if (np > 4096) np = 4096;
        if (cfg.k1_variant != 1 && ME > (u64)4096 * 1400) p.variant = 1;
        p.k1b_ht = ME / np > 600 ? 2048 : 1024;
        if (p.hist && p.k1b_ht == 2048) { p.k1b_ht = 1024; np = std::min<u64>(4096, np * 2); }
    }
    p.np = (u32)np; p.nwg = 256;
    if (ov.np) { const u64 x = uval(ov.np); if (x >= 64 && x <= (narrow ? 2048u : 4096u) && (x & (x - 1)) == 0) p.np = (u32)x; }
    if (ov.ht) { const u64 x = uval(ov.ht); if (x >= 256 && x <= (narrow ? 4096u : 2048u) && (x & (x - 1)) == 0) p.k1b_ht = (u32)x; }
    if (ov.nwg) { const u64 x = uval(ov.nwg); if (x >= 1 && x <= (u64)SG_MAX_K1_WGS) p.nwg = (u32)x; }
    p.pb = 0; while ((1u << p.pb) < p.np) p.pb++;
    if (narrow && 2 * nb - p.pb > 31) { p.np = (u32)np; p.pb = 0; while ((1u << p.pb) < p.np) p.pb++; }
    p.narrow = (narrow && p.variant == 0) ? 1u : 0u;
    if (!p.narrow) p.k1b_split = 1;
    p.warm = (p.narrow && !p.hist && !(cfg.flags & SG_CFG_NO_WARM) && ((cfg.flags & SG_CFG_WARM) || ME >= (1ull << 18))) ? 1u : 0u;
    if (ov.warm) p.warm = (ival(ov.warm) != 0 && p.narrow && !p.hist) ? 1u : 0u;
    p.npb = p.np * p.k1b_split;
    p.nb = nb; p.rb = 2 * nb - p.pb;
    p.pcap = p.narrow ? p.k1b_ht * 13 / 16 : p.k1b_ht * 3 / 4;
    const double m = (double)cfg.max_window_events / ((double)p.np * p.nwg);
    p.sa = std::min<u32>(24, std::max<u32>(8, (2 * 2048 / p.np + 6 + 1) & ~1u));
    if (p.narrow) {
        p.sn = ((u32)(2.0 * m + 8.0 * std::sqrt(m + 1.0) + 24.0) + 1u) & ~1u;
        p.sn = std::min<u32>(p.sn, (1u << 20) - 16);
        p.sw = std::min<u32>(64, std::max<u32>(8, p.sn / 8));
        p.punits = (p.sn + 2 * p.sw + 5 * p.sa + 15) / 16 * 16;
        p.sn = p.punits - 2 * p.sw - 5 * p.sa;
        p.ss = 0; p.pslots = 0;
    } else {
        p.ss = (u32)(2.0 * m + 8.0 * std::sqrt(m + 1.0) + 24.0);
        p.ss = (p.ss + p.agg_slots * p.sa + 7) / 8 * 8 - p.agg_slots * p.sa;
        p.ss = std::min<u32>(p.ss, (1u << 20) - 8);
        p.pslots = p.ss + p.agg_slots * p.sa;
    }
    p.ovf_cap = 1u << 16;
    p.k1b_threads = 1024u;
    if (p.variant == 0)
        p.k1b_lds = p.narrow ? ((size_t)p.k1b_ht * 36 + 8 + (size_t)p.k1b_ht / 4 + 12 + 15) / 16 * 16 : (size_t)p.k1b_ht * (8 + 32 + (p.hist ? 4 * SG_HIST_BINS : 0));
    if (p.narrow) p.k1b_u = 2 * p.k1b_lds > lds && m > 24.0 ? 8 : 4;
    if (ov.k1b_u) { if (ival(ov.k1b_u) == 8) p.k1b_u = 8; if (ival(ov.k1b_u) == 4) p.k1b_u = 4; }
    if (p.k1b_u == 8) p.warm = 0;
    p.k1b_pack = p.narrow && (u64)p.sn * p.nwg < 65536ull;
    if (ov.k1b_pack) { if (ival(ov.k1b_pack) == 0) p.k1b_pack = false; }
    if (ov.k1b_threads) { const u64 x = uval(ov.k1b_threads); if ((x == 256 && !p.narrow) || x == 512 || x == 1024) p.k1b_threads = (u32)x; }
    if (p.narrow && p.k1b_ht / p.k1b_threads > 4) p.k1b_threads = 1024u;
    p.k1b_order = p.narrow && !ov.k1b_no_order;
    p.prepare_fold = p.warm && p.narrow && p.variant == 0 && cfg.world <= 1 && p.k1b_threads == 1024u && p.k1b_lds >= kPrepareLds &&
                     !(ov.no_fold && ival(ov.no_fold) != 0);
    p.max_blocks = p.variant == 0 ? (u32)std::min<u64>(1024, std::max<u64>(64, (u64)cfg.max_ips / 32)) : 2u;
    if (p.variant == 0) p.ecap = K2_TILE;
    p.alive_cap = cfg.max_alive ? cfg.max_alive : 65536u;
    p.kept_edges = p.warm ? std::max<u64>(ME, (u64)p.npb * p.pcap) : ME;
    p.hub_cap = (u32)std::min<u64>(p.kept_edges / 256 + 16, 1u << 24);

    p.k3_ranges = (p.ncap + K3_IN_NR - 1) / K3_IN_NR;
    p.k3_slices = (u32)std::min<u64>((u64)p.k3_ranges * K3_IN_SMAX <= p.cus ? K3_IN_SMAX : 32, std::max<u64>(8, ME / 8192));
    if (ov.k3_slices) { const u64 x = uval(ov.k3_slices); if (x >= 1 && x <= 256) p.k3_slices = (u32)x; }
    p.k3in_lds = (size_t)K3_IN_NR * 48;
    {
        const u64 bw = ((u64)p.ncap + 31) / 32;
        p.k2_sortw = bw <= K2_SORT_LDS ? K2_SORT_LDS : (u32)std::min<u64>(K2_SORT_LDS_MAX, (bw + 255) / 256 * 256);
    }
    {
        u32 g = std::min<u32>(K2_DH_GMAX, p.variant == 0 ? p.npb : 0u);
        if (ME < (1ull << 19)) g = 0;
        if (p.warm) g = 0;
        else if (ov.dh_g) { const u64 x = uval(ov.dh_g); g = (x >= 16 && x <= K2_DH_GMAX && (x & (x - 1)) == 0 && p.variant == 0 && x <= p.npb) ? (u32)x : 0u; }
        if (g >= 16 && (g & (g - 1)) == 0 && p.npb % g == 0 && ((size_t)p.ncap + 1) * sizeof(u32) <= 128u * 1024u && (u64)p.npb * p.pcap < (1ull << 32)) {
            p.dh_g = g; p.dh_ppw = p.npb / g; p.dh_ns = (p.ncap + 1 + 63u) & ~63u;
        }
    }
    p.ablate = ov.ablate ? (u32)std::strtoul(ov.ablate->c_str(), nullptr, 0) : 0u;
    p.k4_split = cfg.max_edges > (1u << 17);
    if (ov.k4_fused) p.k4_split = ival(ov.k4_fused) == 0;
    p.k5_form = k5_form_default(cfg);
    if (ov.k5_form) {
        if (*ov.k5_form != "0" && *ov.k5_form != "1") { if (why) *why = "SG_K5_FORM: 0 (sixteen lanes per edge) or 1 (one lane per edge)"; return SG_EINVAL; }
        p.k5_form = (u32)ival(ov.k5_form);
    }
    if ((u64)p.ncap * 256u > (1ull << 32)) p.k5_form = 0;
    const int k5_per_wg = p.k5_form ? 256 : 32, k5_round = (p.k5_form ? k5_lanes_wgs_per_cu() : 3) * (int)p.cus;
    p.k5_grid = (u32)grid_for(cfg.max_edges, k5_per_wg, k5_round);
    if (ov.k5_grid) { const int x = ival(ov.k5_grid); if (x >= 1 && x <= 65535) p.k5_grid = (u32)std::min(grid_for(cfg.max_edges, k5_per_wg, 65535), x); }
    p.k3_fuse_allowed = !ov.k3_no_fuse;
    p.k6_one_wg = (bool)ov.k6_one_wg;
    if (ov.copy_streams) p.n_copy = ival(ov.copy_streams) == 2 ? 2 : 1;
    if (ov.stage_slots) p.n_stage = std::min(kStageSlots, std::max(2, ival(ov.stage_slots)));
    p.n_slots = std::min<u32>(std::max<u32>(cfg.windows_in_flight, 1), 8);
    *out = p;
    return SG_OK;
}

constexpr bool kK1aPairDefault = true;
inline bool plan_pass_a(const Plan& p, uint32_t l1_entries, size_t l2_bytes, const Overrides& ov, PassA* out) {
    PassA a;
    const size_t lds_cap = kLdsBytes;
    const size_t l1b = (size_t)l1_entries * 8, l2b = l2_bytes;
    const size_t stage_max = (size_t)K1A_NJ * K1A_THREADS * 16;
    if (p.narrow) {
        a.l2_u16 = p.max_known <= 16384 && !ov.l2_u32;
        const size_t l2lds = a.l2_u16 ? l2b / 2 : l2b;
        if (ov.nsub) { const int x = ival(ov.nsub); if (x == 1 || x == 2) a.k1a_nsub = (u32)x; }
        const bool want_tile = ov.k1a && *ov.k1a == "tile", force_team = ov.k1a && *ov.k1a == "team";
        const size_t fixed_tile = (size_t)p.np * 24 + 64 + (size_t)K1T_TS(a.k1a_nsub) * 8 + l1b;
        const int teams = 2, nt = 1024;
        const size_t stage_team = (size_t)K1A_NJ * nt * 16;
        const bool team_ok = (p.np == 256 || p.np == 512 || p.np == 1024) && (size_t)p.np * p.nwg * p.punits * 8 < ((size_t)1 << 31) && l1b <= stage_team;
        a.k1a_teams = (u32)teams; a.k1a_nt = (u32)nt;
        const size_t fixed_team = K1M_LDS_FIXED(p.np, teams, nt) + l1b;
        auto pick = [&](size_t fixed, u32 ct_min, size_t stage_cap, u32& ct, bool& in_lds) {
            ct = 0; in_lds = false;
            for (u32 c : {1024u, 512u, 256u, 128u}) if (c >= ct_min && (size_t)c * 40 + fixed + l2lds <= lds_cap && l1b + l2b <= stage_cap) { in_lds = true; ct = c; break; }
            if (!ct) for (u32 c : {1024u, 512u, 256u, 128u, 64u}) if (c >= ct_min && (size_t)c * 40 + fixed <= lds_cap) { ct = c; break; }
        };
        u32 ct = 0; bool in_lds = false;
        if (!want_tile && team_ok) { pick(fixed_team, force_team ? 64u : 256u, stage_team, ct, in_lds); a.k1a_team = ct != 0; }
        if (!ct) pick(fixed_tile, 64u, stage_max, ct, in_lds);
        const size_t fixed = a.k1a_team ? fixed_team : fixed_tile;
        a.l2_in_lds = in_lds;
        if (ov.l2_global) a.l2_in_lds = false;
        if (ov.ct) { const u32 x = (u32)std::strtoul(ov.ct->c_str(), nullptr, 0); if (x >= 64 && x <= 2048 && (x & (x - 1)) == 0 && (size_t)x * 40 + fixed + (a.l2_in_lds ? l2lds : 0) <= lds_cap) ct = x; }
        if (!ct || l1b > stage_max) return false;
        a.k1a_ct = ct;
        a.k1a_lds = (size_t)ct * 40 + fixed + (a.l2_in_lds ? l2lds : 0);
        {
            const size_t extra = K1M_LDS_PAIR_EXTRA(p.np, teams, nt);
            const bool able = a.k1a_team && 2 * p.nb <= 31 && (p.np == 256 || p.np == 512 || p.np == 1024);
            const bool forced = ov.k1a_pair && ival(ov.k1a_pair) != 0;
            if (able && forced && !ov.ct && ct > 512 && a.k1a_lds + extra > lds_cap && a.k1a_lds - (size_t)(ct - 512) * 40 + extra <= lds_cap) {
                a.k1a_lds -= (size_t)(ct - 512) * 40; ct = 512; a.k1a_ct = ct;
            }
            const bool fits = able && a.k1a_lds + extra <= lds_cap;
            const bool want = ov.k1a_pair ? forced : (kK1aPairDefault && ct >= 512 && p.np <= 512);
            a.k1a_pair = fits && want;
            a.k1a_pair_lds = a.k1a_pair ? extra : 0;
        }
        *out = a;
        return true;
    }
    const size_t fixed = (size_t)p.np * 4 + 64 + l1b;
    const size_t slot = p.hist ? 72 : 40;
    u32 ct = 0;
    for (u32 c : {2048u, 1024u, 512u}) if ((size_t)c * slot + fixed + l2b <= lds_cap && l1b + l2b <= stage_max) { a.l2_in_lds = true; ct = c; break; }
    if (!ct) for (u32 c : {2048u, 1024u, 512u, 256u, 128u, 64u}) if ((size_t)c * slot + fixed <= lds_cap) { ct = c; break; }
    if (ov.ct) { const u32 x = (u32)std::strtoul(ov.ct->c_str(), nullptr, 0); if (x >= 64 && x <= 2048 && (x & (x - 1)) == 0 && (size_t)x * slot + fixed + (a.l2_in_lds ? l2b : 0) <= lds_cap) ct = x; }
    if (ov.l2_global) a.l2_in_lds = false;
    if (!ct || l1b > stage_max) return false;
    a.k1a_ct = ct;
    a.k1a_lds = (size_t)ct * slot + fixed + (a.l2_in_lds ? l2b : 0);
    *out = a;
    return true;
}

enum K1aFamily { K1A_GLOBAL = 0, K1A_WIDE = 1, K1A_TILE = 2, K1A_TEAM = 3 };
enum K1bFamily { K1B_NONE = 0, K1B_MERGE = 1, K1B_STREAM = 2 };
constexpr int kK1bWarmU = 2;
struct PassAKernel {
    int family = K1A_GLOBAL;
    int l2 = 0;
    bool sharded = false, hist = false;
    int nsub = 0, pb = 0;
    bool pair = false;
};
struct Kernels {
    PassAKernel k1a;
    int k1b_family = K1B_NONE, k1b_u = 0, k1b_spt = 0;
    bool k1b_pack = false, k1b_hist = false, k1b_share = false, k1b_warm = false;
    bool k2_dh = false;
    bool k4_split = false, k4_mfma = true;
    bool k5_mfma = true;
    int k5_form = 0;
};
inline PassAKernel choose_pass_a(const Plan& p, const PassA& a, const sg_config& cfg) {
    PassAKernel k;
    if (p.variant != 0) return k;
    k.sharded = cfg.world > 1;
    if (!p.narrow) { k.family = K1A_WIDE; k.l2 = a.l2_in_lds ? 1 : 0; k.hist = p.hist != 0; return k; }
    k.l2 = a.l2_in_lds ? (a.l2_u16 ? 2 : 1) : 0;
    if (a.k1a_team) { k.family = K1A_TEAM; k.pb = p.np == 256 ? 8 : p.np == 512 ? 9 : 10; k.pair = a.k1a_pair; }
    else { k.family = K1A_TILE; k.nsub = a.k1a_nsub == 2 ? 2 : 1; }
    return k;
}
inline Kernels choose_kernels(const Plan& p, const PassA& a, const sg_config& cfg) {
    Kernels k;
    k.k1a = choose_pass_a(p, a, cfg);
    if (p.variant == 0) {
        k.k1b_share = p.npb > p.cus && 2 * p.k1b_lds <= kLdsBytes;
        const u32 spt = p.k1b_ht / p.k1b_threads;
        k.k1b_u = p.k1b_u == 8 ? 8 : 4;
        if (p.warm || p.narrow) { k.k1b_family = K1B_STREAM; k.k1b_spt = spt >= 4 ? 4 : spt == 2 ? 2 : 1; k.k1b_pack = p.k1b_pack; k.k1b_warm = p.warm != 0; }
        else { k.k1b_family = K1B_MERGE; k.k1b_hist = p.hist != 0; if (k.k1b_hist) k.k1b_u = 4; }
    }
    k.k2_dh = p.dh_g != 0;
    k.k4_split = p.k4_split; k.k4_mfma = p.use_mfma; k.k5_mfma = p.use_mfma; k.k5_form = (int)p.k5_form;
    return k;
}

template <size_t N> using Key = std::array<int, N>;
template <size_t... L>
constexpr std::array<Key<sizeof...(L)>, (L * ...)> product(const int (&... v)[L]) {
    std::array<Key<sizeof...(L)>, (L * ...)> out{};
    for (size_t i = 0; i < out.size(); i++) { size_t r = i, k = 0; ((out[i][k++] = v[r % L], r /= L), ...); }
    return out;
}
template <size_t N, size_t A, size_t B>
constexpr std::array<Key<N>, A + B> concat(const std::array<Key<N>, A>& a, const std::array<Key<N>, B>& b) {
    std::array<Key<N>, A + B> out{};
    for (size_t i = 0; i < A; i++) out[i] = a[i];
    for (size_t i = 0; i < B; i++) out[A + i] = b[i];
    return out;
}
template <size_t N, size_t M>
int find_key(const std::array<Key<N>, M>& dom, const Key<N>& k) { for (size_t i = 0; i < M; i++) if (dom[i] == k) return (int)i; return -1; }

inline constexpr auto kK1aWideKeys = product({0, 1}, {0, 1}, {0, 1});
inline constexpr auto kK1aTileKeys = product({0, 1, 2}, {0, 1}, {1, 2});
inline constexpr auto kK1aTeamKeys = product({0, 1, 2}, {0, 1}, {8, 9, 10});
inline constexpr auto kK1aTeamPairKeys = product({0, 1, 2}, {0, 1}, {8, 9, 10});
inline constexpr auto kK1bMergeKeys = concat(product({4, 8}, {0}, {0, 1}), product({4}, {1}, {0, 1}));
inline constexpr auto kK1bStreamKeys = concat(product({4, 8}, {1, 2, 4}, {0, 1}, {0}, {0, 1}),
                                              product({kK1bWarmU}, {1, 2, 4}, {0, 1}, {1, 2}, {0, 1}));
inline constexpr auto kK4LayerKeys = product({32, 64}, {0, 1}, {0, 1}, {0, 1});

constexpr u64 kTrendAlign = 256;
inline u64 trend_align(u64 b) { return (b + kTrendAlign - 1) / kTrendAlign * kTrendAlign; }
struct Piece { const char* name; u64 off, bytes; };
struct Slots { u64 off = 0, bytes = 0; };
struct SlotPiece { const char* name; u64 bytes; u64* rel; };
struct Block {
    u64 align = kTrendAlign, end = 0;
    std::vector<Piece> pieces;
    u64 up(u64 b) const { return (b + align - 1) / align * align; }
    u64 take(const char* name, u64 bytes) {
        const u64 off = up(end);
        pieces.push_back({name, off, bytes});
        end = off + bytes;
        return off;
    }
    Slots slots(u32 n, std::initializer_list<SlotPiece> ps) {
        Slots s;
        for (u32 k = 0; k < std::max<u32>(n, 1); k++) {
            const u64 first = up(end);
            for (const SlotPiece& p : ps) { const u64 off = take(p.name, p.bytes); if (!k) *p.rel = off - first; }
            if (!k) { s.off = first; s.bytes = up(end) - first; }
        }
        return s;
    }
};

constexpr u32 kSelThreads = 256, kSelMaxWgs = 1024, kSelRowsPerWg = 2048, kSelStateWords = 8;
struct SelPlan {
    u32 wgs = 0;
    u64 key_bytes = 0;
    u64 hist_bytes = 0;
    u64 blk_bytes = 0;
    u64 pair_bytes = 0;
    u64 state_bytes = 0;
    u64 scratch_bytes = 0;
    u64 stage_rows = 0;
    u64 pair_off = 0, n_off = 0, state_off = 0, blk_off = 0, hist_off = 0, key_off = 0;
    std::vector<Piece> layout;
};
inline SelPlan plan_select(u64 max_edges, bool used) {
    SelPlan s;
    if (!used) return s;
    s.wgs = (u32)std::max<u64>(1, std::min<u64>(kSelMaxWgs, (max_edges + kSelRowsPerWg - 1) / kSelRowsPerWg));
    s.key_bytes = max_edges * 4;
    s.hist_bytes = (u64)s.wgs * 256 * 4;
    s.blk_bytes = (u64)s.wgs * 4 * 4;
    s.pair_bytes = (u64)SG_SELECT_MAX_K * 8;
    s.state_bytes = kSelStateWords * 4 + 8;
    s.stage_rows = max_edges;
    Block b; b.align = 8;
    s.pair_off = b.take("pairs", s.pair_bytes);
    s.n_off = b.take("state", s.state_bytes); s.state_off = s.n_off + 8;
    s.blk_off = b.take("blk", s.blk_bytes);
    s.hist_off = b.take("hist", s.hist_bytes);
// ... 805 lines not shown
```

alaz_amd/engine.py:

```python
from __future__ import annotations

import ctypes as C
import os
from collections import namedtuple
from typing import Optional, Tuple

import numpy as np

from .replay import EDGE_OUT_DTYPE, EVENT_DTYPE

_HERE = os.path.dirname(os.path.abspath(__file__))
LIB_PATH = os.environ.get("SG_LIB_PATH") or os.path.join(_HERE, "lib", "libservicegraph.so")
LIB_DEV_PATH = os.path.join(_HERE, "lib", "libservicegraph_dev.so")
DEV_KNOBS = ("SG_ABLATE", "SG_NP", "SG_HT", "SG_CT", "SG_NWG", "SG_NSUB", "SG_SPLIT", "SG_WARM", "SG_K1A", "SG_K1_NARROW", "SG_K1_LEGACY", "SG_K1B_U",
             "SG_K1B_THREADS", "SG_K1B_PACK", "SG_K1B_NO_ORDER", "SG_L2_GLOBAL", "SG_L2_U32", "SG_DH_G", "SG_K3_SLICES", "SG_K3_NO_FUSE", "SG_K4_FUSED", "SG_K5_GRID", "SG_K6_ONE_WG", "SG_DENSE_VALU",
             "SG_COPY_STREAMS", "SG_STAGE_SLOTS", "SG_ARENA", "SG_NO_FOLD", "SG_K1A_PAIR", "SG_K5_FORM")

SG_OK, SG_EINVAL, SG_ENOMEM, SG_ENODEV, SG_ENOSPC, SG_EAGAIN, SG_ESTATE = 0, -22, -12, -19, -28, -11, -71
SELECT_MAX_K = 16384
F_IN, F_HID, F_EDGE = 32, 64, 8
STAT_SUM_WORDS, STAT_MAX_WORDS = 12, 2
REF_KNOWN, REF_LABEL, REF_OBIP = 0, 1, 2

TREND_DTYPE = np.dtype([("lat_dev", "<f4"), ("err_dev", "<f4"), ("base_mean_us", "<f4"), ("windows_seen", "<u4")])
TREND_ENTRY_DTYPE = np.dtype([("from_key", "<u8"), ("to_key", "<u8"), ("lat_mean", "<f8"), ("lat_dev", "<f8"), ("err_mean", "<f8"),
                              ("err_dev", "<f8"), ("n", "<u4"), ("last", "<u4")])
NODE_DTYPE = np.dtype([(f"{side}_{f}", "<u8") for f in ("count", "err", "sum_ns", "sumsq_us", "max_ns", "score_q32") for side in ("out", "in")]
                      + [(f, "<u4") for f in ("ref", "out_edges", "in_edges", "out_alive", "in_alive", "out_worst_row", "in_worst_row")]
                      + [(f, "<f4") for f in ("out_score_max", "in_score_max", "score")])
NODE_TREND_DTYPE = np.dtype([(f, "<f4") for f in ("in_lat_dev", "in_err_dev", "out_lat_dev", "out_err_dev", "in_base_mean_us", "out_base_mean_us")]
                            + [("in_seen", "<u4"), ("out_seen", "<u4")])
RANK_DTYPE = np.dtype([("rank", "<u8"), ("ref", "<u4"), ("share", "<f4")])
RANK_SEED = dict(score=0, uniform=1)
RANK_DEFAULTS = dict(iters=0, damping_q8=0, seed="score", seed_min_score=0.0)
INCIDENT_DTYPE = np.dtype([(f, "<u8") for f in ("count", "err", "sum_ns", "score_q32", "rank_sum")]
                          + [(f, "<u4") for f in ("first_node", "nodes", "edges", "worst_row", "top_node", "culprit_node")]
                          + [("value_max", "<f4"), ("reserved", "<u4")])
NO_INCIDENT = 0xFFFFFFFF
INCIDENT_DEFAULTS = dict(by="score", min_value=0.0)
TRACK_DTYPE = np.dtype([(f, "<u4") for f in ("track", "parent", "first_window", "windows", "kept_nodes", "moved_nodes", "joined_nodes", "flags")])
TRACK_ENTRY_DTYPE = np.dtype([(f, "<u4") for f in ("track", "parent", "first_window", "last_window", "windows", "peak_nodes")]
                             + [("count", "<u8"), ("err", "<u8")])
NO_TRACK = 0xFFFFFFFF
TRACK_NEW, TRACK_SPLIT, TRACK_MERGED = 1, 2, 4
TRACK_DEFAULTS = dict(quiet_windows=2, max_tracks=0)
GROUP_EDGE_DTYPE = np.dtype([(f, "<u8") for f in ("count", "err_count", "sum_ns", "sumsq_us", "max_ns", "score_q32")]
                            + [(f, "<u4") for f in ("from_ref", "to_ref", "edges", "from_nodes", "first", "alive", "worst_row")]
                            + [("score_max", "<f4")])
NO_GROUP = 0xFFFFFFFF
REF_GROUP = 3
GROUP_DEFAULTS = dict(max_groups=0)
VANISHED_DTYPE = np.dtype([("from_key", "<u8"), ("to_key", "<u8"), ("lat_mean", "<f8"), ("lat_dev", "<f8"), ("err_mean", "<f8"),
                           ("err_dev", "<f8"), ("n", "<u4"), ("last", "<u4"), ("row", "<u4"), ("reserved", "<u4")])
VANISHED_DEFAULTS = dict(silent_windows=0, min_seen=0, max_rows=0)
SEL_BY = dict(score=0, lat_dev=1, err_dev=2, new=3)
NSEL_BY = dict(score=0, in_lat_dev=1, in_err_dev=2, out_lat_dev=3, out_err_dev=4, new=5)
TREND_DEFAULTS = dict(shift=4, warmup=4, ttl=64, max_entries=0, lat_floor_ns=1000, err_floor=10486)
Q_SPACES = dict(nodes=1, groups=2, group_nodes=4)
Q_MAX = 8
T_SPACES = dict(edges=1, nodes=2, groups=4, group_nodes=8)
TSEL_BY = dict(surge=0, drop=1, load_up=2, load_down=3)
TSEL_SIDE = {"in": 4, "out": 8}
TRAFFIC_DEFAULTS = dict(shift=4, warmup=4, ttl=64, max_entries=0, load_floor_ns=1000000, rate_floor=8)
IMPACT_WORDS = 8
IMPACT_MAX_INCIDENTS = 1024
IMPACT_MAX_HOPS = 64
NO_HOPS = 0xFFFFFFFF
IMPACT_FIELDS = ("exposed", "direct", "far", "entries", "entry_count", "entry_err", "into_count", "into_err")
IMPACT_EXPOSED, IMPACT_DIRECT, IMPACT_FAR, IMPACT_ENTRIES, IMPACT_ENTRY_COUNT, IMPACT_ENTRY_ERR, IMPACT_INTO_COUNT, IMPACT_INTO_ERR = range(8)


class SgConfig(C.Structure):
    _fields_ = [("struct_size", C.c_uint32), ("abi_version", C.c_uint32), ("device", C.c_int32), ("max_known_nodes", C.c_uint32),
                ("max_labels", C.c_uint32), ("max_outbound_ips", C.c_uint32), ("max_ips", C.c_uint32),
                ("max_edges", C.c_uint64), ("max_batch", C.c_uint32), ("layers", C.c_uint32),
                ("rank", C.c_uint32), ("world", C.c_uint32), ("k1_variant", C.c_uint32),
                ("max_window_events", C.c_uint64), ("windows_in_flight", C.c_uint32), ("max_alive", C.c_uint32), ("flags", C.c_uint32)]


CFG_EDGE_HISTOGRAM = 1
CFG_NO_WARM = 2
CFG_WARM = 4
ABI_VERSION = 6


def make_config(*, max_known_nodes: int, max_edges: int, layers: int = 1, max_labels: int = 256, max_outbound_ips: int = 64,
                max_ips: int = 0, max_batch: int = 1 << 16, device: int = 0, rank: int = 0, world: int = 1, k1_variant: int = 0,
                max_window_events: int = 0, windows_in_flight: int = 1, max_alive: int = 0, flags: int = 0) -> "SgConfig":
    return SgConfig(C.sizeof(SgConfig), ABI_VERSION, device, max_known_nodes, max_labels, max_outbound_ips, max_ips or max_known_nodes,
                    max_edges, max_batch, layers, rank, world, k1_variant, max_window_events, windows_in_flight, max_alive, flags)


class SgGeometry(C.Structure):
    _fields_ = [(n, C.c_uint32) for n in ("k1_variant", "k1_narrow", "partitions", "table_slots", "pass_a_workgroups", "cache_slots",
                                          "join_l2_in_lds", "tile_records", "endpoint_bits", "piece_bytes", "pass_b_split", "pass_a_teams", "warm_windows")]


class SgStats(C.Structure):
    _fields_ = [("events_in", C.c_uint64), ("events_dropped_src", C.c_uint64), ("events_dropped_ring", C.c_uint64),
# ... 15 lines not shown
class TrafficParams(C.Structure):
    _fields_ = [("struct_size", C.c_uint32), ("shift", C.c_uint32), ("warmup", C.c_uint32), ("ttl", C.c_uint32),
                ("max_entries", C.c_uint64), ("load_floor_ns", C.c_uint64), ("rate_floor", C.c_uint32), ("reserved", C.c_uint32)]


class SgVanishedParams(C.Structure):
    _fields_ = [("struct_size", C.c_uint32), ("silent_windows", C.c_uint32), ("min_seen", C.c_uint32), ("max_rows", C.c_uint32)]


class SgRankParams(C.Structure):
    _fields_ = [("struct_size", C.c_uint32), ("iters", C.c_uint32), ("damping_q8", C.c_uint32), ("seed", C.c_uint32),
                ("seed_min_score", C.c_float), ("reserved", C.c_uint32)]


class SgIncidentParams(C.Structure):
    _fields_ = [("struct_size", C.c_uint32), ("by", C.c_uint32), ("min_value", C.c_float), ("reserved", C.c_uint32)]


class SgGroupParams(C.Structure):
    _fields_ = [("struct_size", C.c_uint32), ("max_groups", C.c_uint32), ("reserved", C.c_uint32 * 2)]


class SgTrackParams(C.Structure):
    _fields_ = [("struct_size", C.c_uint32), ("quiet_windows", C.c_uint32), ("max_tracks", C.c_uint32), ("reserved", C.c_uint32)]


class SgTrackStats(C.Structure):
    _fields_ = [(n, C.c_uint64) for n in ("windows", "live", "opened", "dropped_cap")]


class SgTrendStats(C.Structure):
    _fields_ = [(n, C.c_uint64) for n in ("windows", "entries", "inserted", "expired", "dropped")]


def _signatures() -> dict:
    I, H, P, PP = C.c_int, C.c_void_p, C.c_void_p, C.POINTER(C.c_void_p)
    u32, u64, sz, f32 = C.c_uint32, C.c_uint64, C.c_size_t, C.c_float
    Psz, Pu64, Pf64 = C.POINTER(sz), C.POINTER(u64), C.POINTER(C.c_double)
    return {
        "sg_abi_version": (u32, []), "sg_weights_count": (sz, [u32]), "sg_hash32": (u32, [u32]),
        "sg_last_error": (C.c_char_p, [H]),
        "sg_create": (I, [C.POINTER(SgConfig), PP]), "sg_destroy": (I, [H]),
        "sg_upsert_pod": (I, [H, u32, u32]), "sg_delete_pod": (I, [H, u32]),
        "sg_upsert_service": (I, [H, u32, u32]), "sg_delete_service": (I, [H, u32]),
        "sg_set_clock": (I, [H, u64, u64]), "sg_set_label_count": (I, [H, u32]),
        "sg_load_weights": (I, [H, P, sz]),
        "sg_ingest": (I, [H, P, sz]), "sg_ingest_device": (I, [H, P, sz, P]),
        "sg_flush_window": (I, [H, u64, P, sz, Psz]),
        "sg_flush_window_view": (I, [H, u64, PP, Psz]),
        "sg_flush_begin": (I, [H, u64]),
        "sg_flush_end": (I, [H, P, sz, Psz]),
        "sg_flush_end_view": (I, [H, PP, Psz]),
        "sg_window_run": (I, [H, P]), "sg_window_rows_buffer": (I, [H, PP]),
        "sg_window_close": (I, [H, P]),
        "sg_window_obip_list": (I, [H, P, u32, P, P]),
        "sg_bind_buffers": (I, [H, P, P, PP, u32]),
        "sg_window_close_sharded": (I, [H, P, P, P]),
        "sg_window_features": (I, [H, P]), "sg_window_layer": (I, [H, u32, P]),
        "sg_window_score": (I, [H, P]), "sg_window_score_reset": (I, [H, P]), "sg_window_read": (I, [H, P, sz, Psz]),
        "sg_window_reset": (I, [H, P]),
        "sg_window_buffers": (I, [H, PP, PP, PP, Psz]),
        "sg_window_feat_buffer": (I, [H, u32, PP, Psz]),
        "sg_halo_build": (I, [H, P, u32, P, P]), "sg_halo_pack": (I, [H, u32, P, u32, P, P]),
        "sg_halo_unpack": (I, [H, u32, P, u32, P, P]),
        "sg_window_close_gathered": (I, [H, P, u32, u32, P]),
        "sg_halo_build_padded": (I, [H, P, u32, P]), "sg_halo_pack_padded": (I, [H, u32, P, u32, P, P]),
        "sg_halo_unpack_padded": (I, [H, u32, P, u32, P, P]),
        "sg_window_outbound_ips": (I, [H, P, sz, Psz]),
        "sg_stats_get": (I, [H, C.POINTER(SgStats)]),
        "sg_timing_enable": (I, [H, I]), "sg_timing_reset": (I, [H]),
        "sg_timing_get": (I, [H, I, Pf64, Pu64]),
        "sg_set_warm": (I, [H, I]), "sg_timing_stride": (I, [H, u32]),
        "sg_timing_samples": (I, [H, I, Pf64, sz, Psz]),
        "sg_latency_probe": (I, [H, u64, u32, I, Pf64]),
        "sg_debug_stamps": (I, [H, P, sz]),
        "sg_clock_probe": (I, [H, u32, Pf64, Pf64]),
        "sg_comm_probe": (I, []), "sg_window_halo_counts": (I, [H, P, sz]),
        "sg_route": (I, [H, P, sz, u32, P]),
        "sg_window_hist": (I, [H, P, sz, Psz]),
        "sg_geometry_get": (I, [H, C.POINTER(SgGeometry)]),
        "sg_prepare_fold_get": (I, [H, C.POINTER(u32)]),
        "sg_pass_a_pair_get": (I, [H, C.POINTER(u32)]),
        "sg_k5_form_get": (I, [H, C.POINTER(u32)]),
        "sg_comm_unique_id": (I, [P, sz]), "sg_comm_create": (I, [P, sz, I, I, I, PP]),
        "sg_comm_destroy": (I, [P]), "sg_window_run_sharded": (I, [H, P, P]),
        "sg_host_register": (I, [H, P, sz]), "sg_host_unregister": (I, [H, P]), "sg_ingest_pinned": (I, [H, P, sz]),
        "sg_ingest_bulk": (I, [H, P, sz, I, Pu64]),
        "sg_flush_window_top": (I, [H, u64, u32, f32, P, P, sz, Psz, Psz]),
        "sg_flush_end_top": (I, [H, u32, f32, P, P, sz, Psz, Psz]),
        "sg_window_select": (I, [H, u32, f32, P, P, sz, P, P]),
        "sg_set_trend": (I, [H, P]), "sg_window_trend": (I, [H, P, sz, P, sz, Psz]),
        "sg_window_trend_buffer": (I, [H, PP]), "sg_trend_entries": (I, [H, P, sz, Psz]),
        "sg_trend_stats_get": (I, [H, P]),
        "sg_set_nodes": (I, [H, I]), "sg_window_nodes": (I, [H, P, sz, Psz]),
        "sg_window_nodes_buffer": (I, [H, PP, PP]),
        "sg_set_vanished": (I, [H, P]), "sg_window_vanished": (I, [H, P, sz, Psz]),
        "sg_window_vanished_buffer": (I, [H, PP, PP]),
        "sg_flush_window_top_by": (I, [H, u64, u32, u32, f32, P, P, sz, Psz, Psz]),
        "sg_flush_end_top_by": (I, [H, u32, u32, f32, P, P, sz, Psz, Psz]),
        "sg_window_select_by": (I, [H, u32, u32, f32, P, P, sz, P, P]),
        "sg_set_node_trend": (I, [H, P]), "sg_window_node_trend": (I, [H, P, sz, P, sz, Psz]),
        "sg_window_node_trend_buffer": (I, [H, PP]), "sg_node_trend_entries": (I, [H, P, sz, Psz]),
        "sg_node_trend_stats_get": (I, [H, P]),
        "sg_window_nodes_top": (I, [H, u32, u32, f32, P, P, sz, Psz, Psz]),
        "sg_window_nodes_select": (I, [H, u32, u32, f32, P, P, sz, P, P]),
        "sg_set_rank": (I, [H, P]), "sg_window_rank": (I, [H, P, sz, P, sz, Psz]),
        "sg_window_rank_buffer": (I, [H, PP]),
        "sg_window_rank_top": (I, [H, u32, f32, P, P, P, sz, Psz, Psz]),
        "sg_window_rank_select": (I, [H, u32, f32, P, P, sz, P, P]),
        "sg_set_incidents": (I, [H, P]), "sg_window_incidents": (I, [H, P, sz, Psz]),
        "sg_window_node_incident": (I, [H, P, sz, P, sz, Psz]),
        "sg_window_incidents_buffer": (I, [H, PP, PP, PP]),
        "sg_set_tracks": (I, [H, P]), "sg_window_incident_tracks": (I, [H, P, sz, Psz]),
        "sg_window_tracks_ended": (I, [H, P, sz, Psz]),
        "sg_window_tracks_buffer": (I, [H, PP, PP, PP]),
        "sg_track_entries": (I, [H, P, sz, Psz]), "sg_track_stats_get": (I, [H, P]),
        "sg_set_groups": (I, [H, P]), "sg_group_assign": (I, [H, P, P, sz]),
        "sg_window_groups": (I, [H, P, sz, Psz]), "sg_window_row_group": (I, [H, P, sz, P, sz, Psz]),
        "sg_window_group_perm": (I, [H, P, sz, Psz]),
        "sg_window_groups_buffer": (I, [H] + [PP] * 4),
        "sg_set_group_trend": (I, [H, P]), "sg_window_group_trend": (I, [H, P, sz, P, sz, Psz]),
        "sg_window_group_trend_buffer": (I, [H, PP]), "sg_group_trend_entries": (I, [H, P, sz, Psz]),
        "sg_group_trend_stats_get": (I, [H, P]),
        "sg_set_group_vanished": (I, [H, P]), "sg_window_group_vanished": (I, [H, P, sz, Psz]),
        "sg_window_group_vanished_buffer": (I, [H, PP, PP]),
        "sg_window_groups_top": (I, [H, u32, u32, f32, P, P, sz, Psz, Psz]),
        "sg_window_groups_select": (I, [H, u32, u32, f32, P, P, sz, P, P]),
        "sg_set_group_nodes": (I, [H, I]), "sg_window_group_nodes": (I, [H, P, sz, Psz]),
        "sg_window_group_nodes_buffer": (I, [H, PP, PP]),
        "sg_set_group_node_trend": (I, [H, P]), "sg_window_group_node_trend": (I, [H, P, sz, P, sz, Psz]),
        "sg_window_group_node_trend_buffer": (I, [H, PP]), "sg_group_node_trend_entries": (I, [H, P, sz, Psz]),
        "sg_group_node_trend_stats_get": (I, [H, P]),
        "sg_window_group_nodes_top": (I, [H, u32, u32, f32, P, P, sz, Psz, Psz]),
        "sg_window_group_nodes_select": (I, [H, u32, u32, f32, P, P, sz, P, P]),
        "sg_set_group_rank": (I, [H, P]), "sg_window_group_rank": (I, [H, P, sz, P, sz, Psz]),
        "sg_window_group_rank_buffer": (I, [H, PP]),
        "sg_window_group_rank_top": (I, [H, u32, f32, P, P, P, sz, Psz, Psz]),
        "sg_window_group_rank_select": (I, [H, u32, f32, P, P, sz, P, P]),
        "sg_set_group_incidents": (I, [H, P]), "sg_window_group_incidents": (I, [H, P, sz, Psz]),
        "sg_window_group_node_incident": (I, [H, P, sz, P, sz, Psz]),
        "sg_window_group_incidents_buffer": (I, [H, PP, PP, PP]),
        "sg_set_group_tracks": (I, [H, P]), "sg_window_group_incident_tracks": (I, [H, P, sz, Psz]),
        "sg_window_group_tracks_ended": (I, [H, P, sz, Psz]),
        "sg_window_group_tracks_buffer": (I, [H, PP, PP, PP]),
        "sg_group_track_entries": (I, [H, P, sz, Psz]), "sg_group_track_stats_get": (I, [H, P]),
        "sg_set_group_impact": (I, [H, u32, u32]), "sg_window_group_impact": (I, [H, P, sz, Psz]),
        "sg_window_group_node_hops": (I, [H, P, sz, P, sz, Psz]),
        "sg_window_group_impact_mask": (I, [H, P, sz, Psz, C.POINTER(u32)]),
        "sg_window_group_impact_buffer": (I, [H, PP, PP, PP, PP]),
        "sg_set_quantiles": (I, [H, u32, P, sz]),
        "sg_window_node_hist": (I, [H, P, sz, P, sz, Psz]), "sg_window_node_quantiles": (I, [H, P, sz, P, sz, Psz]),
        "sg_window_group_hist": (I, [H, P, sz, P, sz, Psz]), "sg_window_group_quantiles": (I, [H, P, sz, P, sz, Psz]),
        "sg_window_group_node_hist": (I, [H, P, sz, P, sz, Psz]), "sg_window_group_node_quantiles": (I, [H, P, sz, P, sz, Psz]),
        "sg_window_quantiles_buffer": (I, [H, u32, PP, PP]),
        "sg_set_quantile_trend": (I, [H, u32, u32, P]),
        "sg_window_node_quantile_trend": (I, [H, P, sz, P, sz, Psz]), "sg_window_group_quantile_trend": (I, [H, P, sz, P, sz, Psz]),
        "sg_window_group_node_quantile_trend": (I, [H, P, sz, P, sz, Psz]),
        "sg_window_quantile_trend_buffer": (I, [H, u32, PP]),
        "sg_quantile_trend_entries": (I, [H, u32, P, sz, Psz]), "sg_quantile_trend_stats_get": (I, [H, u32, P]),
        "sg_window_nodes_top_tail": (I, [H, u32, u32, f32, P, P, sz, Psz, Psz]),
        "sg_window_groups_top_tail": (I, [H, u32, u32, f32, P, P, sz, Psz, Psz]),
        "sg_window_group_nodes_top_tail": (I, [H, u32, u32, f32, P, P, sz, Psz, Psz]),
        "sg_set_traffic_trend": (I, [H, u32, P]),
        "sg_window_traffic": (I, [H, P, sz, P, sz, Psz]), "sg_window_node_traffic": (I, [H, P, sz, P, sz, Psz]),
        "sg_window_group_traffic": (I, [H, P, sz, P, sz, Psz]), "sg_window_group_node_traffic": (I, [H, P, sz, P, sz, Psz]),
        "sg_window_traffic_buffer": (I, [H, u32, PP]),
# ... 151 lines not shown
            if kw:
                raise TypeError(f"{st.off} and takes no parameters")
            self._ck(call(self._h, *lead, None))
            return None
        v = dict(st.defaults)
        v.update(params or {}); v.update(kw)
        unknown = set(v) - {f for f, _ in st.struct._fields_}
        if unknown:
            raise TypeError(f"unknown {st.noun} parameters: {sorted(unknown)}")
        p = st.struct(struct_size=C.sizeof(st.struct))
        for f, x in v.items():
            setattr(p, f, st.convert[f](x) if f in st.convert else x)
        self._ck(call(self._h, *lead, C.byref(p)))
        return v

    def _counted(self, call, dtype, shape_tail=()) -> np.ndarray:
        n = C.c_size_t(0)
        self._ck(call(self._h, None, 0, C.byref(n)))
        out = np.zeros((n.value,) + shape_tail, dtype=dtype)
        if n.value:
            self._ck(call(self._h, out.ctypes.data, n.value, C.byref(n)))
        return out[: n.value]

    def _window_rows(self, call, dtype, index):
        if index is None:
            return self._counted(lambda h, out, cap, n: call(h, None, 0, out, cap, n), dtype)
        idx = np.ascontiguousarray(index, dtype=np.uint32)
        out = np.zeros(len(idx), dtype=dtype)
        if len(idx):
            self._ck(call(self._h, idx.ctypes.data, len(idx), out.ctypes.data, len(idx), C.byref(C.c_size_t(0))))
        return out

    def _capped(self, call, cap: Optional[int]) -> np.ndarray:
        cap = self.max_edges if cap is None else cap
        out = np.zeros(cap, dtype=EDGE_OUT_DTYPE); n = C.c_size_t(0)
        self._ck(call(out.ctypes.data, cap, C.byref(n)))
        return out[: min(n.value, cap)]

    def _top(self, call, cap: int, *dtypes):
        outs = [np.zeros(cap, dtype=d) for d in dtypes]
        ns, nt = C.c_size_t(0), C.c_size_t(0)
        self._ck(call(*[o.ctypes.data for o in outs], cap, C.byref(ns), C.byref(nt)))
        m = min(ns.value, cap)
        return (*[o[:m] for o in outs], nt.value)

    def _node_cap(self, k: int, cap: Optional[int], count=None) -> int:
        if cap is not None:
            return cap
        if k:
            return k
        n = C.c_size_t(0)
        self._ck((count or self._l.sg_window_nodes)(self._h, None, 0, C.byref(n)))
        return n.value

    def _pointers(self, call, n: int) -> tuple:
        p = [C.c_void_p() for _ in range(n)]
        self._ck(call(self._h, *[C.byref(x) for x in p]))
        return tuple(x.value for x in p)

    def _stats(self, call, struct):
        s = struct()
        self._ck(call(self._h, C.byref(s)))
        return s

    def close(self):
        if getattr(self, "_h", None):
            self._l.sg_destroy(self._h); self._h = None

    def __del__(self):
        try:
            self.close()
        except Exception:
            pass

    def geometry(self) -> dict:
        g = SgGeometry()
        self._ck(self._l.sg_geometry_get(self._h, C.byref(g)))
        fold = C.c_uint32(0)
        self._ck(self._l.sg_prepare_fold_get(self._h, C.byref(fold)))
        pair = C.c_uint32(0)
        self._ck(self._l.sg_pass_a_pair_get(self._h, C.byref(pair)))
        form = C.c_uint32(0)
        self._ck(self._l.sg_k5_form_get(self._h, C.byref(form)))
        return {**{n: int(getattr(g, n)) for n, _ in SgGeometry._fields_}, "prepare_fold": int(fold.value), "pass_a_pair": int(pair.value), "k5_form": int(form.value)}

    def k1_kernels(self) -> tuple:
        g = self.geometry()
        if g["k1_variant"] == 1: return ("k1_resolve_aggregate",)
        if not g["k1_narrow"]: return ("k1a_partition", "k1b_merge")
        return ("k1a_team_partition" if g["pass_a_teams"] else "k1a_tile_partition", "k1b_stream_merge")

    def upsert_pod(self, ip: int, node_id: int): self._ck(self._l.sg_upsert_pod(self._h, ip, node_id))
    def delete_pod(self, ip: int): self._ck(self._l.sg_delete_pod(self._h, ip))
    def upsert_service(self, ip: int, node_id: int): self._ck(self._l.sg_upsert_service(self._h, ip, node_id))
    def delete_service(self, ip: int): self._ck(self._l.sg_delete_service(self._h, ip))
    def set_clock(self, first_kernel_ns: int, first_user_ns: int): self._ck(self._l.sg_set_clock(self._h, first_kernel_ns, first_user_ns))
    def set_label_count(self, n: int): self._ck(self._l.sg_set_label_count(self._h, n))

    def load_weights(self, w: np.ndarray):
        w = np.ascontiguousarray(w, dtype=np.float32)
        self._ck(self._l.sg_load_weights(self._h, w.ctypes.data, len(w)))

    def ingest(self, events: np.ndarray) -> int:
        ev = np.ascontiguousarray(events)
        assert ev.dtype == EVENT_DTYPE
        return self._ck(self._l.sg_ingest(self._h, ev.ctypes.data, len(ev)), allow=(SG_EAGAIN,))

    def host_register(self, arr: np.ndarray):
        assert arr.flags.c_contiguous
        self._ck(self._l.sg_host_register(self._h, arr.ctypes.data, arr.nbytes))

    def host_unregister(self, arr: np.ndarray): self._ck(self._l.sg_host_unregister(self._h, arr.ctypes.data))

    def ingest_pinned(self, events: np.ndarray) -> int:
        assert events.dtype == EVENT_DTYPE and events.flags.c_contiguous
        return self._ck(self._l.sg_ingest_pinned(self._h, events.ctypes.data, len(events)), allow=(SG_EAGAIN,))

    def ingest_bulk(self, events: np.ndarray, pinned: bool = False) -> int:
        assert events.dtype == EVENT_DTYPE and events.flags.c_contiguous
        w = C.c_uint64(0)
        self._ck(self._l.sg_ingest_bulk(self._h, events.ctypes.data, len(events), 1 if pinned else 0, C.byref(w)))
        return int(w.value)

    def ingest_device(self, dev_ptr: int, n: int, stream: int = 0):
        self._ck(self._l.sg_ingest_device(self._h, dev_ptr, n, stream or None))

    def flush_window(self, window_end_ms: int = 0, cap: Optional[int] = None) -> np.ndarray:
        return self._capped(lambda out, c, n: self._l.sg_flush_window(self._h, window_end_ms, out, c, n), cap)

    def flush_window_view(self, window_end_ms: int = 0) -> np.ndarray:
        ptr = C.c_void_p(); n = C.c_size_t(0)
        self._ck(self._l.sg_flush_window_view(self._h, window_end_ms, C.byref(ptr), C.byref(n)))
        return self._rows_view(ptr, n)

    def flush_begin(self, window_end_ms: int = 0):
        self._ck(self._l.sg_flush_begin(self._h, window_end_ms))

    def flush_end_view(self) -> np.ndarray:
        ptr = C.c_void_p(); n = C.c_size_t(0)
        self._ck(self._l.sg_flush_end_view(self._h, C.byref(ptr), C.byref(n)))
        return self._rows_view(ptr, n)

    def flush_end(self, cap: int | None = None) -> np.ndarray:
        return self._capped(lambda out, c, n: self._l.sg_flush_end(self._h, out, c, n), cap)

    @staticmethod
    def _by(by) -> int:
        if by not in SEL_BY:
            raise ValueError(f"by must be one of {sorted(SEL_BY)}, not {by!r}")
        return SEL_BY[by]

    def flush_window_top(self, k: int, min_score: float = float("-inf"), window_end_ms: int = 0, cap: Optional[int] = None,
                         by: str = "score"):
        b = self._by(by)
        cap = (k or self.max_edges) if cap is None else cap
        if b:
            return self._top(lambda *a: self._l.sg_flush_window_top_by(self._h, window_end_ms, b, k, min_score, *a), cap, EDGE_OUT_DTYPE, np.uint32)
        return self._top(lambda *a: self._l.sg_flush_window_top(self._h, window_end_ms, k, min_score, *a), cap, EDGE_OUT_DTYPE, np.uint32)

    def flush_end_top(self, k: int, min_score: float = float("-inf"), cap: Optional[int] = None, by: str = "score"):
        b = self._by(by)
        cap = (k or self.max_edges) if cap is None else cap
        if b:
            return self._top(lambda *a: self._l.sg_flush_end_top_by(self._h, b, k, min_score, *a), cap, EDGE_OUT_DTYPE, np.uint32)
        return self._top(lambda *a: self._l.sg_flush_end_top(self._h, k, min_score, *a), cap, EDGE_OUT_DTYPE, np.uint32)

    def window_select(self, k: int, min_score: float, d_out: int, d_index: int, cap: int, d_n: int, stream: int = 0, by: str = "score"):
# ... 538 lines not shown
```

include/servicegraph.h:

```cpp
#ifndef SERVICEGRAPH_H
#define SERVICEGRAPH_H

#include <stddef.h>
#include <stdint.h>

#ifdef __cplusplus
extern "C" {
#endif

#define SG_ABI_VERSION 6u

#define SG_OK        0
#define SG_EINVAL   (-22)
#define SG_ENOMEM   (-12)
#define SG_ENODEV   (-19)
#define SG_ENOSPC   (-28)
#define SG_EAGAIN   (-11)
#define SG_ESTATE   (-71)

#define SG_PROTO_UNKNOWN  0
#define SG_PROTO_HTTP     1
#define SG_PROTO_AMQP     2
#define SG_PROTO_POSTGRES 3
#define SG_PROTO_HTTP2    4
// ... 425 lines not shown
    uint32_t reserved;
} sg_traffic_params;
int sg_set_traffic_trend(sg_handle h, uint32_t spaces, const sg_traffic_params* p);
int sg_window_traffic(sg_handle h, const uint32_t* row_index, size_t n_index, sg_edge_trend* out, size_t cap, size_t* n);
int sg_window_node_traffic(sg_handle h, const uint32_t* node_index, size_t n_index, sg_node_trend* out, size_t cap, size_t* n);
int sg_window_group_traffic(sg_handle h, const uint32_t* group_index, size_t n_index, sg_edge_trend* out, size_t cap, size_t* n);
int sg_window_group_node_traffic(sg_handle h, const uint32_t* node_index, size_t n_index, sg_node_trend* out, size_t cap, size_t* n);
int sg_window_traffic_buffer(sg_handle h, uint32_t space, void** d_rows);
int sg_traffic_trend_entries(sg_handle h, uint32_t space, sg_trend_entry* out, size_t cap, size_t* n);
int sg_traffic_trend_stats_get(sg_handle h, uint32_t space, sg_trend_stats* out);
#define SG_TSEL_SURGE      0u
#define SG_TSEL_DROP       1u
#define SG_TSEL_LOAD_UP    2u
#define SG_TSEL_LOAD_DOWN  3u
#define SG_TSEL_IN         4u
#define SG_TSEL_OUT        8u
int sg_window_nodes_top_traffic(sg_handle h, uint32_t by, uint32_t k, float min_value, sg_node_out* out, uint32_t* node_index, size_t cap, size_t* n_selected, size_t* n_nodes);
int sg_window_groups_top_traffic(sg_handle h, uint32_t by, uint32_t k, float min_value, sg_group_edge* out, uint32_t* group_index, size_t cap, size_t* n_selected, size_t* n_groups);
int sg_window_group_nodes_top_traffic(sg_handle h, uint32_t by, uint32_t k, float min_value, sg_node_out* out, uint32_t* node_index, size_t cap, size_t* n_selected, size_t* n_nodes);

int sg_flush_begin(sg_handle h, uint64_t window_end_ms);
int sg_flush_end(sg_handle h, sg_edge_out* out, size_t cap, size_t* n);
int sg_flush_end_view(sg_handle h, const sg_edge_out** rows, size_t* n);

int sg_window_run(sg_handle h, void* stream);
int sg_window_rows_buffer(sg_handle h, void** d_rows);

int sg_window_close(sg_handle h, void* stream);
int sg_window_obip_list(sg_handle h, uint32_t* d_list, uint32_t cap, uint32_t* d_n, void* stream);
int sg_window_close_sharded(sg_handle h, const uint32_t* d_union_ips, const uint32_t* d_union_n, void* stream);
int sg_window_close_gathered(sg_handle h, const uint32_t* d_gathered, uint32_t stride, uint32_t world, void* stream);
int sg_window_features(sg_handle h, void* stream);
int sg_window_layer(sg_handle h, uint32_t l, void* stream);
int sg_window_score(sg_handle h, void* stream);
int sg_window_score_reset(sg_handle h, void* stream);
int sg_window_read(sg_handle h, sg_edge_out* out, size_t cap, size_t* n);
int sg_window_reset(sg_handle h, void* stream);

int sg_window_buffers(sg_handle h, void** stats_sum, void** stats_max, void** counters,
                      size_t* n_nodes_cap);
int sg_window_feat_buffer(sg_handle h, uint32_t l, void** rows, size_t* row_floats);

int sg_bind_buffers(sg_handle h, void* stats_sum, void* stats_max, void* const* feat_rows, uint32_t n_feat);

int sg_halo_build(sg_handle h, uint32_t* d_ids, uint32_t cap, uint32_t* d_counts, void* stream);
int sg_halo_build_padded(sg_handle h, uint32_t* d_req, uint32_t capp, void* stream);
int sg_halo_pack_padded(sg_handle h, uint32_t l, const uint32_t* d_serve, uint32_t capp, float* d_rows, void* stream);
int sg_halo_unpack_padded(sg_handle h, uint32_t l, const uint32_t* d_req, uint32_t capp, const float* d_rows, void* stream);
int sg_halo_pack(sg_handle h, uint32_t l, const uint32_t* d_ids, uint32_t n, float* d_rows, void* stream);
int sg_halo_unpack(sg_handle h, uint32_t l, const uint32_t* d_ids, uint32_t n, const float* d_rows, void* stream);

typedef struct sg_comm sg_comm;
int sg_comm_probe(void);
int sg_comm_unique_id(void* id128, size_t bytes);
int sg_comm_create(const void* id128, size_t bytes, int rank, int world, int device, sg_comm** out);
int sg_comm_destroy(sg_comm* c);
int sg_window_run_sharded(sg_handle h, sg_comm* comm, void* stream);
int sg_window_halo_counts(sg_handle h, uint32_t* counts, size_t world);

int sg_window_outbound_ips(sg_handle h, uint32_t* ips, size_t cap, size_t* n);
int sg_window_hist(sg_handle h, uint32_t* bins, size_t cap_rows, size_t* n);

int sg_stats_get(sg_handle h, sg_stats* out);

typedef struct sg_geometry {
    uint32_t k1_variant;
    uint32_t k1_narrow;
    uint32_t partitions;
    uint32_t table_slots;
    uint32_t pass_a_workgroups;
    uint32_t cache_slots;
    uint32_t join_l2_in_lds;
    uint32_t tile_records;
    uint32_t endpoint_bits;
    uint32_t piece_bytes;
    uint32_t pass_b_split;
    uint32_t pass_a_teams;
    uint32_t warm_windows;
} sg_geometry;
int sg_geometry_get(sg_handle h, sg_geometry* out);
int sg_prepare_fold_get(sg_handle h, uint32_t* out);
int sg_pass_a_pair_get(sg_handle h, uint32_t* out);
int sg_k5_form_get(sg_handle h, uint32_t* out);

int sg_timing_enable(sg_handle h, int on);
int sg_timing_reset(sg_handle h);
int sg_timing_stride(sg_handle h, uint32_t n);
int sg_timing_get(sg_handle h, int kernel, double* avg_us, uint64_t* launches);
int sg_set_warm(sg_handle h, int on);
int sg_timing_samples(sg_handle h, int kernel, double* us, size_t cap, size_t* n);
int sg_latency_probe(sg_handle h, uint64_t bytes, uint32_t steps, int warm, double* ns_per_load);
int sg_clock_probe(sg_handle h, uint32_t spin_us, double* spin_mhz, double* k1a_mhz);
int sg_debug_stamps(sg_handle h, uint64_t* out, size_t n);

uint32_t sg_hash32(uint32_t x);
int sg_route(sg_handle h, const sg_event* events, size_t n, uint32_t world, uint32_t* shard_out);

#ifdef __cplusplus
}
#endif
#endif
```

Measured before the change: 23.75 billion events/s.

## Compute edge features inside lane-form edge scorer instead of storing them in k3

Moves per-edge feature computation (log counts, mean/sd latency, z-score, error ratio) from k3_node_features into k5_edge_score_lanes. The scorer now computes them from acc_csr and row stats it prefetches for the next batch, and the efeat/latz/errr buffers are no longer allocated. This removes a full write and re-read of the 8-float edge feature arrays plus two scalar arrays over all edges. In exchange the scorer does more VALU and double-precision math and holds more registers, and it reads lane IDs through an opaque asm barrier, which may hurt occupancy or scheduling.

```diff
diff --git a/alaz_amd/csrc/servicegraph.hip b/alaz_amd/csrc/servicegraph.hip
--- a/alaz_amd/csrc/servicegraph.hip
+++ b/alaz_amd/csrc/servicegraph.hip
@@ -266,7 +266,8 @@
 constexpr K2RowptrFn kK2Rowptr[2] = {k2_rowptr<K2_RP_ROWS, false>, k2_rowptr<K2_RP_ROWS_DH, true>};
 constexpr K4GatherFn kK4Gather[2] = {k4_gather<32>, k4_gather<64>};
 constexpr K5ProjFn kK5Proj[2] = {k5_node_proj<false>, k5_node_proj<true>};
-constexpr K5ScoreFn kK5Score[2][2] = {{k5_edge_score<false>, k5_edge_score<true>}, {k5_edge_score_lanes<false>, k5_edge_score_lanes<true>}};
+constexpr K5ScoreFn kK5Score[2][2][2] = {{{k5_edge_score<false>, k5_edge_score<true>}, {k5_edge_score_lanes<false, false>, k5_edge_score_lanes<true, false>}},
+                                         {{nullptr, nullptr}, {k5_edge_score_lanes<false, true>, k5_edge_score_lanes<true, true>}}};
 static_assert(sgplan::kK5LanesWgLds == 4 * K5L_WAVE_LDS, "sg_plan.hpp's copy of form 1's LDS per workgroup");
 template <class F, size_t... I>
 const std::array<typename F::Fn, sizeof...(I)>& kernel_table(std::index_sequence<I...>) {
@@ -563,7 +564,7 @@
 int do_features(sg_engine* e, hipStream_t s) {
     const Dev& d = work(e).d;
     Timed t(e, s, 3);
-    const int nbn = grid_for(d.ncap, 128), nbe = grid_for(e->cfg.max_edges, 256, 4096);
+    const int nbn = grid_for(d.ncap, 128), nbe = e->plan.k5_efeat ? 0 : grid_for(e->cfg.max_edges, 256, 4096);
     hipLaunchKernelGGL(k3_node_features, dim3(nbn + nbe), dim3(256), 0, s, d, (u32)nbn, e->in_fused_slices);
     e->in_fused_slices = 0;
     HIP_TRY(e, hipGetLastError());
@@ -1237,7 +1238,7 @@
     {
         Timed t(e, s, 5);
         if (!(proj_done && d.world == 1)) hipLaunchKernelGGL(e->fn.k5_proj, dim3(grid_for(d.ncap, 16)), dim3(256), 0, s, d, d.h[e->cfg.layers], Wh);
-        hipLaunchKernelGGL(kK5Score[e->kn.k5_form][fr], dim3((int)e->plan.k5_grid), dim3(256), 0, s, d, Wh);
+        hipLaunchKernelGGL(kK5Score[e->kn.k5_efeat][e->kn.k5_form][fr], dim3((int)e->plan.k5_grid), dim3(256), 0, s, d, Wh);
     }
     if (did_reset) *did_reset = fr;
     HIP_TRY(e, hipGetLastError());
@@ -2126,7 +2127,7 @@
         LR(dev_alloc(e, &w.P, (size_t)w.ncap * SG_F_HID)); LR(dev_alloc(e, &w.Q, (size_t)w.ncap * SG_F_HID));
         LR(dev_alloc(e, &w.nmean, (size_t)w.ncap * SG_F_HID));
         LR(dev_alloc(e, &w.hub_items, w.hub_cap)); LR(dev_alloc(e, &w.hub_base, (size_t)w.ncap + 1)); LR(dev_alloc(e, &w.hub_part, (size_t)w.hub_cap * SG_F_HID));
-        LR(dev_alloc(e, &w.efeat, ME * SG_F_EDGE)); LR(dev_alloc(e, &w.latz, ME)); LR(dev_alloc(e, &w.errr, ME));
+        if (!P.k5_efeat) { LR(dev_alloc(e, &w.efeat, ME * SG_F_EDGE)); LR(dev_alloc(e, &w.latz, ME)); LR(dev_alloc(e, &w.errr, ME)); }
         LR(dev_alloc(e, &w.row_mu, (size_t)w.ncap + 1)); LR(dev_alloc(e, &w.row_sd, (size_t)w.ncap + 1));
         LR(dev_alloc(e, &w.rows, ME));
         LR(dev_alloc(e, &w.in_part, (size_t)P.k3_ranges * P.k3_slices * K3_IN_NR * 6));
@@ -2226,6 +2227,13 @@
     if (!e || !out) return SG_EINVAL;
     std::lock_guard<std::mutex> g(e->mu);
     *out = (uint32_t)e->kn.k5_form;
+    return SG_OK;
+}
+
+int sg_k5_efeat_get(sg_handle e, uint32_t* out) {
+    if (!e || !out) return SG_EINVAL;
+    std::lock_guard<std::mutex> g(e->mu);
+    *out = (uint32_t)e->kn.k5_efeat;
     return SG_OK;
 }
 
diff --git a/alaz_amd/csrc/sg_k2.h b/alaz_amd/csrc/sg_k2.h
--- a/alaz_amd/csrc/sg_k2.h
+++ b/alaz_amd/csrc/sg_k2.h
@@ -495,26 +495,45 @@
     const double sm = x * (1.0 - x * (0.5 - x * (1.0 / 3.0 - 0.25 * x)));
     return x < 1e-4 ? sm : r;
 }
-__device__ __forceinline__ void edge_features(const Dev& d, u32 pos) {
-    const ulonglong2* a = reinterpret_cast<const ulonglong2*>(d.acc_csr + (size_t)pos * 4);
-    const ulonglong2 x = a[0], y = a[1];
-    const u32 from = d.csr_from[pos];
+template <class RowStats, class Out>
+__device__ __forceinline__ void edge_feature_values(const Dev& d, const ulonglong2 x, const ulonglong2 y, RowStats row_stats, Out& out) {
     const u64 cnt = x.x & 0xFFFFFFFFull, err = x.x >> 32, sum = x.y, mx = y.x, ssq = y.y;
     const double rc = cnt ? sg_rcp((double)cnt) : 0.0, dc = (double)cnt;
     const double sum_us = (double)sum * 1e-3;
     double m_e = sum_us * rc; m_e = cnt ? fma(fma(-dc, m_e, sum_us), rc, m_e) : 0.0;
     double q_e = (double)ssq * rc; q_e = cnt ? fma(fma(-dc, q_e, (double)ssq), rc, q_e) : 0.0;
     const double var = q_e - m_e * m_e, s_e = var > 0.0 ? sqrt(var) : 0.0;
-    const double mu = d.row_mu[from], sd = d.row_sd[from];
+    double mu, sd; row_stats(mu, sd);
     const double z = sd > 1.0 ? sg_div(m_e - mu, sd) : m_e - mu;
     const float lat_z = (float)z;
     const float err_ratio = !cnt ? 0.0f : ((cnt | err) < (1ull << 24) ? (float)(u32)err / (float)(u32)cnt : (float)((double)err / (double)cnt));
     const float zc = lat_z < -8.0f ? -8.0f : (lat_z > 8.0f ? 8.0f : lat_z);
-    float4* e = reinterpret_cast<float4*>(d.efeat + (size_t)pos * SG_F_EDGE);
-    e[0] = make_float4(log1p_count(d, cnt), (float)sg_log1p_pos(m_e * 1e-3), (float)sg_log1p_pos(s_e * 1e-3), (float)sg_log1p_pos((double)mx * 1e-6));
-    e[1] = make_float4(err_ratio, log1p_count(d, err), zc * 0.125f, 1.0f);
-    d.latz[pos] = lat_z; d.errr[pos] = err_ratio;
-}
+    out.begin();
+    out.e0(make_float4(log1p_count(d, cnt), (float)sg_log1p_pos(m_e * 1e-3), (float)sg_log1p_pos(s_e * 1e-3), (float)sg_log1p_pos((double)mx * 1e-6)));
+    out.e1(make_float4(err_ratio, log1p_count(d, err), zc * 0.125f, 1.0f));
+    out.tail(lat_z, err_ratio);
+}
+struct EdgeFeatStore {
+    const Dev& d; u32 pos; float4* e;
+    __device__ __forceinline__ void begin() { e = reinterpret_cast<float4*>(d.efeat + (size_t)pos * SG_F_EDGE); }
+    __device__ __forceinline__ void e0(float4 v) const { e[0] = v; }
+    __device__ __forceinline__ void e1(float4 v) const { e[1] = v; }
+    __device__ __forceinline__ void tail(float lat_z, float err_ratio) const { d.latz[pos] = lat_z; d.errr[pos] = err_ratio; }
+};
+__device__ __forceinline__ void edge_features(const Dev& d, u32 pos) {
+    const ulonglong2* a = reinterpret_cast<const ulonglong2*>(d.acc_csr + (size_t)pos * 4);
+    const ulonglong2 x = a[0], y = a[1];
+    const u32 from = d.csr_from[pos];
+    EdgeFeatStore out{d, pos, nullptr};
+    edge_feature_values(d, x, y, [&](double& mu, double& sd) { mu = d.row_mu[from]; sd = d.row_sd[from]; }, out);
+}
+struct EdgeFeat {
+    float4 w0, w1; float lat_z, err_ratio;
+    __device__ __forceinline__ void begin() {}
+    __device__ __forceinline__ void e0(float4 v) { w0 = v; }
+    __device__ __forceinline__ void e1(float4 v) { w1 = v; }
+    __device__ __forceinline__ void tail(float z, float r) { lat_z = z; err_ratio = r; }
+};
 
 #define K2_LONG_WGS 1024
 #define K2_WAVE_ROW 512
diff --git a/alaz_amd/csrc/sg_k5.h b/alaz_amd/csrc/sg_k5.h
--- a/alaz_amd/csrc/sg_k5.h
+++ b/alaz_amd/csrc/sg_k5.h
@@ -186,7 +186,7 @@
 #define K5L_WAVE_LDS 8192u
 __device__ __forceinline__ void k5l_lds_order() { __builtin_amdgcn_fence(__ATOMIC_ACQ_REL, "wavefront"); __builtin_amdgcn_wave_barrier(); }
 
-template <bool RESET>
+template <bool RESET, bool EFEAT>
 __global__ __launch_bounds__(256) __attribute__((amdgpu_waves_per_eu(3))) void k5_edge_score_lanes(Dev d, const float* __restrict__ Wh) {
 #pragma clang fp contract(off)
     static_assert(SG_F_HID == 64 && SG_F_EDGE == 8, "k5_edge_score_lanes: 64 hidden units in four quarters, eight edge features");
@@ -205,15 +205,20 @@
         const u32 rx = (lane >> 2) & 3u;
         const u32 ox = (lane >> 1) & 3u;
         const u32 rb = (((lane >> 3) * 4 + (((lane & 7u) >> 1) ^ ((lane >> 4) & 3u))) << 1) | (lane & 1u);
+        auto relane = [&]() -> u32 { u32 l = lane; asm volatile("" : "+v"(l)); return l; };
         u32 gu[4], gv[4];
         f32x4 R[8];
         auto load_ids = [&](u32 p0) {
-#pragma unroll
-            for (int i = 0; i < 4; i++) { const u32 p = p0 + i * 16 + sub, c = p < E ? p : last; gu[i] = d.csr_from[c]; gv[i] = d.col[c]; }
+            u32 subl = 0;
+            if constexpr (EFEAT) subl = relane() >> 2;
+#pragma unroll
+            for (int i = 0; i < 4; i++) { const u32 p = EFEAT ? p0 + i * 16 + subl : p0 + i * 16 + sub, c = p < E ? p : last; gu[i] = d.csr_from[c]; gv[i] = d.col[c]; }
         };
         auto row_offsets = [&]() {
-#pragma unroll
-            for (int i = 0; i < 4; i++) { gu[i] = gu[i] * (SG_F_HID * 4u) + pc * 16u; gv[i] = gv[i] * (SG_F_HID * 4u) + pc * 16u; }
+            u32 pc_ = pc;
+            if constexpr (EFEAT) pc_ = relane() & 3u;
+#pragma unroll
+            for (int i = 0; i < 4; i++) { gu[i] = gu[i] * (SG_F_HID * 4u) + pc_ * 16u; gv[i] = gv[i] * (SG_F_HID * 4u) + pc_ * 16u; }
         };
         auto issue = [&](int c) {
 #pragma unroll
@@ -226,8 +231,10 @@
         float ek[SG_F_EDGE];
         auto quarter = [&](int c, float (&out)[4]) {
             f32x4 pq[4];
-#pragma unroll
-            for (int w = 0; w < 4; w++) pq[w] = tile[(lane * 4 + rx) ^ (u32)w] + tile[256 + ((lane * 4 + rx) ^ (u32)w)];
+            u32 rd = lane * 4 + rx;
+            if (EFEAT) { const u32 l = relane(); rd = l * 4 + ((l >> 2) & 3u); }
+#pragma unroll
+            for (int w = 0; w < 4; w++) pq[w] = tile[rd ^ (u32)w] + tile[256 + (rd ^ (u32)w)];
             f32x4 W[2][4], w2v[4];
             auto wload = [&](int blk, f32x4 (&dst)[4]) {
                 u32 o = (u32)((blk & 1) * 4 * SG_F_HID + 16 * (blk >> 1) + 4 * c);
@@ -267,26 +274,45 @@
             out[0] = sa.x; out[1] = sa.y; out[2] = sb.x; out[3] = sb.y;
         };
         u32 b = wave;
-        if (b < nbatch) { load_ids(b * 64u); row_offsets(); issue(0); }
+        u32 nfrom = 0; ulonglong2 nx = {0, 0}, ny = {0, 0}; double nmu = 0.0, nsd = 0.0;
+        auto load_own = [&](u32 c) {
+            nx = reinterpret_cast<const ulonglong2*>(d.acc_csr + (size_t)c * 4)[0]; ny = reinterpret_cast<const ulonglong2*>(d.acc_csr + (size_t)c * 4)[1];
+            nmu = d.row_mu[nfrom]; nsd = d.row_sd[nfrom];
+        };
+        if (b < nbatch) {
+            if (EFEAT) { const u32 c0 = b * 64u + lane < E ? b * 64u + lane : last; nfrom = d.csr_from[c0]; load_own(c0); }
+            load_ids(b * 64u); row_offsets(); issue(0);
+        }
         for (; b < nbatch; b += nw) {
             const u32 p0 = b * 64u;
             const u32 er = p0 + lane, ec = er < E ? er : last;
             const u32 np0 = b + nw < nbatch ? (b + nw) * 64u : last;
-            const f32x4 e0 = reinterpret_cast<const f32x4*>(d.efeat + (size_t)ec * SG_F_EDGE)[0], e1 = reinterpret_cast<const f32x4*>(d.efeat + (size_t)ec * SG_F_EDGE)[1];
+            const u32 nec = EFEAT ? (np0 + lane < E ? np0 + lane : last) : 0u;
+            f32x4 e0, e1; u32 wer, wlz;
+            if (!EFEAT) { e0 = reinterpret_cast<const f32x4*>(d.efeat + (size_t)ec * SG_F_EDGE)[0]; e1 = reinterpret_cast<const f32x4*>(d.efeat + (size_t)ec * SG_F_EDGE)[1]; }
             float T[4];
 #define K5L_STAGE(C, NEXT) { k5l_lds_order();                                                                                \
-                _Pragma("unroll") for (int i = 0; i < 4; i++) { tile[64 * i + wslot] = R[i]; tile[256 + 64 * i + wslot] = R[4 + i]; } \
+                u32 ws_ = wslot; if (EFEAT) { const u32 l = relane(), s_ = l >> 2; ws_ = s_ * 4 + ((l & 3u) ^ ((s_ >> 2) & 3u)); }           \
+                _Pragma("unroll") for (int i = 0; i < 4; i++) { tile[64 * i + ws_] = R[i]; tile[256 + 64 * i + ws_] = R[4 + i]; } \
                 k5l_lds_order(); NEXT; __builtin_amdgcn_sched_barrier(0); }
-            K5L_STAGE(0, issue(2))
+            auto features = [&]() {
+                EdgeFeat f;
+                edge_feature_values(d, nx, ny, [&](double& mu_, double& sd_) { mu_ = nmu; sd_ = nsd; }, f);
+                e0 = (f32x4){ f.w0.x, f.w0.y, f.w0.z, f.w0.w }; e1 = (f32x4){ f.w1.x, f.w1.y, f.w1.z, f.w1.w };
+                wlz = __float_as_uint(f.lat_z); wer = __float_as_uint(f.err_ratio);
+                __builtin_amdgcn_sched_barrier(0);
+            };
+            K5L_STAGE(0, { if (EFEAT) features(); issue(2); })
             ek[0] = e0[0]; ek[1] = e0[1]; ek[2] = e0[2]; ek[3] = e0[3]; ek[4] = e1[0]; ek[5] = e1[1]; ek[6] = e1[2]; ek[7] = e1[3];
             { float o[4]; quarter(0, o); S[0] = o[0]; S[1] = o[1]; S[2] = o[2]; S[3] = o[3]; }
             K5L_STAGE(2, issue(1))
             { float o[4]; quarter(2, o); for (int i = 0; i < 4; i++) S[i] = S[i] + o[i]; }
-            K5L_STAGE(1, { issue(3); load_ids(np0); })
+            K5L_STAGE(1, { issue(3); load_ids(np0); if (EFEAT) nfrom = d.csr_from[nec]; })
             { float o[4]; quarter(1, o); S[4] = o[0]; S[5] = o[1]; S[6] = o[2]; S[7] = o[3]; }
             const ulonglong2 a01 = reinterpret_cast<const ulonglong2*>(d.acc_csr + (size_t)ec * 4)[0], a23 = reinterpret_cast<const ulonglong2*>(d.acc_csr + (size_t)ec * 4)[1];
             const u32 mu = d.csr_from[ec], mv = d.col[ec];
-            const u32 wer = reinterpret_cast<const u32*>(d.errr)[ec], wlz = reinterpret_cast<const u32*>(d.latz)[ec], wal = d.alive_csr[ec];
+            if (!EFEAT) { wer = reinterpret_cast<const u32*>(d.errr)[ec]; wlz = reinterpret_cast<const u32*>(d.latz)[ec]; }
+            const u32 wal = d.alive_csr[ec];
             K5L_STAGE(3, { row_offsets(); issue(0); })
             { float o[4]; quarter(3, o); for (int i = 0; i < 4; i++) S[4 + i] = S[4 + i] + o[i]; }
 #undef K5L_STAGE
@@ -298,12 +324,15 @@
             const u64 refs = (u64)ref_of_dense(mu, nk, nl) | ((u64)ref_of_dense(mv, nk, nl) << 32);
             u64 pct = 0;
             if (d.hist) pct = k5_percentiles(d, ec, (u32)(a01.x & 0xFFFFFFFFull), a23.x);
+            if (EFEAT) load_own(nec);
             v4u_t* const ot = reinterpret_cast<v4u_t*>(tile);
+            u32 ln = lane, ox_ = ox, rb_ = rb;
+            if (EFEAT) { ln = relane(); ox_ = (ln >> 1) & 3u; rb_ = (((ln >> 3) * 4 + (((ln & 7u) >> 1) ^ ((ln >> 4) & 3u))) << 1) | (ln & 1u); }
             k5l_lds_order();
-            ot[(lane * 4 + ox) ^ 0u] = (v4u_t){ (u32)a01.y, (u32)(a01.y >> 32), (u32)a23.x, (u32)(a23.x >> 32) };
-            ot[(lane * 4 + ox) ^ 1u] = (v4u_t){ (u32)a23.y, (u32)(a23.y >> 32), (u32)refs, (u32)(refs >> 32) };
-            ot[(lane * 4 + ox) ^ 2u] = (v4u_t){ (u32)a01.x, (u32)(a01.x >> 32), score, wlz };
-            ot[(lane * 4 + ox) ^ 3u] = (v4u_t){ wer, wal, (u32)pct, (u32)(pct >> 32) };
+            ot[(ln * 4 + ox_) ^ 0u] = (v4u_t){ (u32)a01.y, (u32)(a01.y >> 32), (u32)a23.x, (u32)(a23.x >> 32) };
+            ot[(ln * 4 + ox_) ^ 1u] = (v4u_t){ (u32)a23.y, (u32)(a23.y >> 32), (u32)refs, (u32)(refs >> 32) };
+            ot[(ln * 4 + ox_) ^ 2u] = (v4u_t){ (u32)a01.x, (u32)(a01.x >> 32), score, wlz };
+            ot[(ln * 4 + ox_) ^ 3u] = (v4u_t){ wer, wal, (u32)pct, (u32)(pct >> 32) };
             k5l_lds_order();
             {
                 const u32 p0u = (u32)__builtin_amdgcn_readfirstlane((int)p0);
@@ -311,7 +340,7 @@
                 const __amdgpu_buffer_rsrc_t rr_ = __builtin_amdgcn_make_buffer_rsrc(reinterpret_cast<u64*>(d.rows) + (size_t)p0u * 8, 0, (int)(nrow * 64u), 0x00020000);
                 const v2u_t* const rt = reinterpret_cast<const v2u_t*>(tile);
 #pragma unroll
-                for (int j = 0; j < 8; j++) __builtin_amdgcn_raw_buffer_store_b64(rt[64 * j + rb], rr_, (u32)j * 512u + lane * 8u, 0, 0);
+                for (int j = 0; j < 8; j++) __builtin_amdgcn_raw_buffer_store_b64(rt[64 * j + rb_], rr_, (u32)j * 512u + ln * 8u, 0, 0);
             }
         }
     }
diff --git a/alaz_amd/csrc/sg_plan.hpp b/alaz_amd/csrc/sg_plan.hpp
--- a/alaz_amd/csrc/sg_plan.hpp
+++ b/alaz_amd/csrc/sg_plan.hpp
@@ -36,7 +36,7 @@
 struct Overrides {
     typedef std::optional<std::string> Knob;
     Knob ablate, np, ht, ct, nwg, nsub, split, warm, k1a, k1_narrow, k1_legacy, k1b_u, k1b_threads, k1b_pack, k1b_no_order,
-         l2_global, l2_u32, dh_g, k3_slices, k3_no_fuse, k4_fused, k5_grid, k6_one_wg, dense_valu, copy_streams, stage_slots, arena, no_fold, k1a_pair, k5_form;
+         l2_global, l2_u32, dh_g, k3_slices, k3_no_fuse, k4_fused, k5_grid, k6_one_wg, dense_valu, copy_streams, stage_slots, arena, no_fold, k1a_pair, k5_form, k5_efeat;
 };
 struct KnobName { const char* name; Overrides::Knob Overrides::*field; };
 constexpr KnobName kKnobs[] = {
@@ -49,7 +49,7 @@
     {"SG_K4_FUSED", &Overrides::k4_fused}, {"SG_K5_GRID", &Overrides::k5_grid}, {"SG_K6_ONE_WG", &Overrides::k6_one_wg},
     {"SG_DENSE_VALU", &Overrides::dense_valu}, {"SG_COPY_STREAMS", &Overrides::copy_streams}, {"SG_STAGE_SLOTS", &Overrides::stage_slots},
     {"SG_ARENA", &Overrides::arena}, {"SG_NO_FOLD", &Overrides::no_fold}, {"SG_K1A_PAIR", &Overrides::k1a_pair},
-    {"SG_K5_FORM", &Overrides::k5_form},
+    {"SG_K5_FORM", &Overrides::k5_form}, {"SG_K5_EFEAT", &Overrides::k5_efeat},
 };
 #ifdef SG_DEV_KNOBS
 inline Overrides from_env() {
@@ -78,6 +78,7 @@
     bool k4_split = false;
     u32 k5_grid = 0;
     u32 k5_form = 0;
+    u32 k5_efeat = 0;
     bool k3_fuse_allowed = true;
     bool k6_one_wg = false;
     bool use_mfma = true;
@@ -114,6 +115,7 @@
 
 constexpr u64 kK5LanesMinEdges = 1ull << 20;
 inline u32 k5_form_default(const sg_config& cfg) { return cfg.world <= 1 && cfg.max_edges >= kK5LanesMinEdges ? 1u : 0u; }
+constexpr bool kK5EfeatDefault = true;
 constexpr size_t kK5LanesWgLds = 4 * 8192;
 constexpr int kK5LanesWaves = 3;
 constexpr int k5_lanes_wgs_per_cu() { return (int)std::min<size_t>(kLdsBytes / kK5LanesWgLds, (size_t)kK5LanesWaves); }
@@ -235,6 +237,12 @@
         p.k5_form = (u32)ival(ov.k5_form);
     }
     if ((u64)p.ncap * 256u > (1ull << 32)) p.k5_form = 0;
+    p.k5_efeat = p.k5_form && kK5EfeatDefault ? 1u : 0u;
+    if (ov.k5_efeat) {
+        if (*ov.k5_efeat != "0" && *ov.k5_efeat != "1") { if (why) *why = "SG_K5_EFEAT: 0 (k3_node_features stores the edge features) or 1 (k5_edge_score_lanes computes them)"; return SG_EINVAL; }
+        p.k5_efeat = (u32)ival(ov.k5_efeat);
+        if (p.k5_efeat && !p.k5_form) { if (why) *why = "SG_K5_EFEAT=1 needs form 1 of k5_edge_score (SG_K5_FORM)"; return SG_EINVAL; }
+    }
     const int k5_per_wg = p.k5_form ? 256 : 32, k5_round = (p.k5_form ? k5_lanes_wgs_per_cu() : 3) * (int)p.cus;
     p.k5_grid = (u32)grid_for(cfg.max_edges, k5_per_wg, k5_round);
     if (ov.k5_grid) { const int x = ival(ov.k5_grid); if (x >= 1 && x <= 65535) p.k5_grid = (u32)std::min(grid_for(cfg.max_edges, k5_per_wg, 65535), x); }
@@ -326,6 +334,7 @@
     bool k4_split = false, k4_mfma = true;
     bool k5_mfma = true;
     int k5_form = 0;
+    int k5_efeat = 0;
 };
 inline PassAKernel choose_pass_a(const Plan& p, const PassA& a, const sg_config& cfg) {
     PassAKernel k;
@@ -348,7 +357,7 @@
         else { k.k1b_family = K1B_MERGE; k.k1b_hist = p.hist != 0; if (k.k1b_hist) k.k1b_u = 4; }
     }
     k.k2_dh = p.dh_g != 0;
-    k.k4_split = p.k4_split; k.k4_mfma = p.use_mfma; k.k5_mfma = p.use_mfma; k.k5_form = (int)p.k5_form;
+    k.k4_split = p.k4_split; k.k4_mfma = p.use_mfma; k.k5_mfma = p.use_mfma; k.k5_form = (int)p.k5_form; k.k5_efeat = (int)p.k5_efeat;
     return k;
 }
 
diff --git a/alaz_amd/engine.py b/alaz_amd/engine.py
--- a/alaz_amd/engine.py
+++ b/alaz_amd/engine.py
@@ -14,7 +14,7 @@
 LIB_DEV_PATH = os.path.join(_HERE, "lib", "libservicegraph_dev.so")
 DEV_KNOBS = ("SG_ABLATE", "SG_NP", "SG_HT", "SG_CT", "SG_NWG", "SG_NSUB", "SG_SPLIT", "SG_WARM", "SG_K1A", "SG_K1_NARROW", "SG_K1_LEGACY", "SG_K1B_U",
              "SG_K1B_THREADS", "SG_K1B_PACK", "SG_K1B_NO_ORDER", "SG_L2_GLOBAL", "SG_L2_U32", "SG_DH_G", "SG_K3_SLICES", "SG_K3_NO_FUSE", "SG_K4_FUSED", "SG_K5_GRID", "SG_K6_ONE_WG", "SG_DENSE_VALU",
-             "SG_COPY_STREAMS", "SG_STAGE_SLOTS", "SG_ARENA", "SG_NO_FOLD", "SG_K1A_PAIR", "SG_K5_FORM")
+             "SG_COPY_STREAMS", "SG_STAGE_SLOTS", "SG_ARENA", "SG_NO_FOLD", "SG_K1A_PAIR", "SG_K5_FORM", "SG_K5_EFEAT")
 
 SG_OK, SG_EINVAL, SG_ENOMEM, SG_ENODEV, SG_ENOSPC, SG_EAGAIN, SG_ESTATE = 0, -22, -12, -19, -28, -11, -71
 SELECT_MAX_K = 16384
@@ -196,6 +196,7 @@
         "sg_prepare_fold_get": (I, [H, C.POINTER(u32)]),
         "sg_pass_a_pair_get": (I, [H, C.POINTER(u32)]),
         "sg_k5_form_get": (I, [H, C.POINTER(u32)]),
+        "sg_k5_efeat_get": (I, [H, C.POINTER(u32)]),
         "sg_comm_unique_id": (I, [P, sz]), "sg_comm_create": (I, [P, sz, I, I, I, PP]),
         "sg_comm_destroy": (I, [P]), "sg_window_run_sharded": (I, [H, P, P]),
         "sg_host_register": (I, [H, P, sz]), "sg_host_unregister": (I, [H, P]), "sg_ingest_pinned": (I, [H, P, sz]),
@@ -513,7 +514,10 @@
         self._ck(self._l.sg_pass_a_pair_get(self._h, C.byref(pair)))
         form = C.c_uint32(0)
         self._ck(self._l.sg_k5_form_get(self._h, C.byref(form)))
-        return {**{n: int(getattr(g, n)) for n, _ in SgGeometry._fields_}, "prepare_fold": int(fold.value), "pass_a_pair": int(pair.value), "k5_form": int(form.value)}
+        efeat = C.c_uint32(0)
+        self._ck(self._l.sg_k5_efeat_get(self._h, C.byref(efeat)))
+        return {**{n: int(getattr(g, n)) for n, _ in SgGeometry._fields_}, "prepare_fold": int(fold.value), "pass_a_pair": int(pair.value), "k5_form": int(form.value),
+                "k5_efeat": int(efeat.value)}
 
     def k1_kernels(self) -> tuple:
         g = self.geometry()
diff --git a/include/servicegraph.h b/include/servicegraph.h
--- a/include/servicegraph.h
+++ b/include/servicegraph.h
@@ -531,6 +531,7 @@
 int sg_prepare_fold_get(sg_handle h, uint32_t* out);
 int sg_pass_a_pair_get(sg_handle h, uint32_t* out);
 int sg_k5_form_get(sg_handle h, uint32_t* out);
+int sg_k5_efeat_get(sg_handle h, uint32_t* out);
 
 int sg_timing_enable(sg_handle h, int on);
 int sg_timing_reset(sg_handle h);
```

Measured after the change: 24.19 billion events/s, median of 6. 1.02x the previous value.
